# TuringLang/AdvancedVI.jl

Measured on AMD Instinct MI355X. Metric: ELBO-grad-estimates/sec, higher is better.
Workload: dtype f32

## Files before the change

advancedvi.jl_amd/csrc/api_batch.hip:

```cpp
#include "api_common.h"

mivi_status_t begin_capture(mivi_ctx *c, hipStream_t *saved) {
  if (!c->cap_stream) HIPCHK(c, hipStreamCreateWithFlags(&c->cap_stream, hipStreamNonBlocking));

  HIPCHK(c, hipStreamSynchronize(c->stream));
  *saved = c->stream;
  c->stream = c->cap_stream;
  hipError_t e = hipStreamBeginCapture(c->cap_stream, hipStreamCaptureModeThreadLocal);
  if (e != hipSuccess) { c->stream = *saved; c->err = std::string("hipStreamBeginCapture: ") + hipGetErrorString(e); return MIVI_ERR_HIP; }
  return MIVI_OK;
}
hipError_t end_capture(mivi_ctx *c, hipStream_t saved, hipGraph_t *graph) {
  hipError_t e = hipStreamEndCapture(c->cap_stream, graph);
  c->stream = saved;
  return e;
}

bool graph_capturable(const mivi_ctx *c) {
  return c->target == TGT_DIAG_GAUSS || c->target == TGT_DENSE_GAUSS || c->target == TGT_FUNNEL || c->target == TGT_LOGREG;
}
mivi_status_t reserve_target(mivi_ctx *c, int M) {
  if (c->target == TGT_LOGREG && !logreg_reserve(c, M)) return fail(c, MIVI_ERR_HIP, "logistic regression: scratch allocation failed");
  return MIVI_OK;
}

static mivi_status_t estimate_gradient_chain(mivi_ctx *c, const void *params, uint64_t idx0, int32_t count, void *value, void *grad) {
  if (!c || !params || !value || !grad || count <= 0) return MIVI_ERR_BAD_ARG;
  const uint64_t st = (uint64_t)c->idx_stride;
  if (!graph_capturable(c)) return fail(c, MIVI_ERR_UNSUPPORTED, "graph batching needs a device-resident built-in target");
  if (c->idx_src) return fail(c, MIVI_ERR_UNSUPPORTED, "an index source is set (mivi_set_index_source): graph-batched calls keep their own device counter");
  (void)hipSetDevice(c->cfg.device);
  mivi_status_t s = ensure_work(c, c->cfg.n_mc);
  if (s) return s;
  prepare_tables(c, c->cfg.n_mc);
  if ((s = reserve_target(c, c->cfg.n_mc))) return s;
  static const bool no_fused_loop_n = getenv("MIVI_NO_FUSED_LOOP") != nullptr;
  if (c->cfg.family == MIVI_MEANFIELD && c->target == TGT_DIAG_GAUSS && !c->bij_on && c->cfg.n_mc <= 4096 && !c->idx_src && !no_fused_loop_n) {
    const size_t hist_doubles = (size_t)count * 4 * (size_t)((c->cfg.d + 3) / 4);
    const size_t lane_bytes = (size_t)mf_loop_lanes(c, count) * 2 * (size_t)c->cfg.d * c->esize;
    if ((s = ensure(c, c->X, ((size_t)count + hist_doubles + 8) * sizeof(double) + lane_bytes, false))) return s;
    double *rec = (double *)c->X.p;
    launch_mf_sgd_loop(c, const_cast<void *>(params), nullptr, idx0, 0, count, -1, 0.0, (double)NAN, rec + count, rec, grad,
                       (void *)(rec + count + hist_doubles + 8), value);
    HIPCHK(c, hipGetLastError());
    return MIVI_OK;
  }
  if (c->cfg.family == MIVI_MEANFIELD && c->target == TGT_FUNNEL && !c->funnel_constrained && !c->bij_on && c->cfg.n_mc <= 256 && !c->idx_src &&
      !no_fused_loop_n) {
    const size_t d4 = (size_t)((c->cfg.d + 3) / 4);
    const size_t nd = (size_t)count * 6 * d4 + (size_t)count + 8;
    const size_t sc_bytes = ((size_t)count * ((size_t)c->cfg.d + 2) * c->esize + 63) & ~(size_t)63;
    const size_t lane_bytes = (size_t)mf_loop_lanes(c, count) * 2 * (size_t)c->cfg.d * c->esize;
    const size_t lane_al = (lane_bytes + 63) & ~(size_t)63;
    const size_t e0_bytes = (size_t)count * (size_t)c->cfg.n_mc * c->esize;
    if ((s = ensure(c, c->X, nd * sizeof(double) + sc_bytes + lane_al + e0_bytes + 64, false))) return s;
    double *hist = (double *)c->X.p, *elbo = hist + (size_t)count * 6 * d4;
    void *scratch = (void *)(elbo + count + 8);
    launch_mf_funnel_loop(c, params, idx0, count, hist, elbo, scratch, value, grad, (void *)((char *)scratch + sc_bytes),
                          (void *)((char *)scratch + sc_bytes + lane_al));
    HIPCHK(c, hipGetLastError());
    return MIVI_OK;
  }
  static const int graph_min = getenv("MIVI_GRAPH_MIN") ? atoi(getenv("MIVI_GRAPH_MIN")) : 6;
  if (count < graph_min && c->cfg.family == MIVI_FULLRANK) {
    Chain chn;
    chn.on = true;
    chn.estimates_only = true;
    for (int i = 0; i < count && s == MIVI_OK; ++i) {
      c->cur = i & 1;
      chn.has_next = (i + 1 < count);
      chn.next_rng = rng_of(c, idx0 + ((uint64_t)i + 1) * st);
      s = run_estimate(c, params, rng_of(c, idx0 + (uint64_t)i * st), c->cfg.n_mc, 1, final_out(c, value, grad), &chn);
    }
    if (s == MIVI_OK) flush_chain(c, params, &chn);
    c->cur = 0;
    c->pre_valid = false;
    if (s) return s;
    HIPCHK(c, hipGetLastError());
    return MIVI_OK;
  }
  GraphCache &g = c->graph;
  if (!(g.exec && g.kind == 1 && g.count == count && g.params == params && g.value == value && g.grad == grad)) {
    invalidate_graph(c);
    hipGraph_t graph = nullptr;
    hipStream_t saved;
    if ((s = begin_capture(c, &saved))) return s;
    Chain chn;
    chn.on = true;
    chn.estimates_only = true;
    for (int i = 0; i < count && s == MIVI_OK; ++i) {
      RngArgs r = rng_of(c, (uint64_t)i * st);
      r.idx_ptr = (const uint64_t *)c->d_idx.p;
      c->cur = i & 1;
      chn.has_next = (i + 1 < count);
      chn.next_rng = rng_of(c, ((uint64_t)i + 1) * st);
      chn.next_rng.idx_ptr = r.idx_ptr;
      s = run_estimate(c, params, r, c->cfg.n_mc, 1, final_out(c, value, grad), &chn);
    }
    if (s == MIVI_OK) flush_chain(c, params, &chn);
    if (s == MIVI_OK) hipLaunchKernelGGL(k_bump_u64, dim3(1), dim3(1), 0, c->stream, (uint64_t *)c->d_idx.p, (uint64_t)count * st);
    c->cur = 0;
    hipError_t e = end_capture(c, saved, &graph);
    if (s) { if (graph) (void)hipGraphDestroy(graph); return s; }
    HIPCHK(c, e);
    HIPCHK(c, hipGraphInstantiate(&g.exec, graph, nullptr, nullptr, 0));
    (void)hipGraphDestroy(graph);
    g.kind = 1; g.count = count; g.params = params; g.value = value; g.grad = grad;
  }
  if (!(c->d_idx_valid && c->d_idx_expect == idx0))
    hipLaunchKernelGGL(k_set_u64x2, dim3(1), dim3(1), 0, c->stream, (uint64_t *)c->d_idx.p, idx0, 0ull, 1);
  HIPCHK(c, hipGraphLaunch(g.exec, c->stream));
  c->d_idx_valid = true;
  c->d_idx_expect = idx0 + (uint64_t)count * st;
  return MIVI_OK;
}

static int chain_lanes() {
  static const int v = getenv("MIVI_CHAINS") ? atoi(getenv("MIVI_CHAINS")) : 0;
  return v;
}
mivi_status_t sync_kid(mivi_ctx *c, mivi_ctx *k, int lanes) {
  if (k->kid_gen == c->target_gen && k->idx_stride == lanes) return MIVI_OK;
  invalidate_graph(k);
  k->target = c->target;
  k->t_const = c->t_const;
  k->t_mean = c->t_mean; k->t_istd = c->t_istd; k->t_prec = c->t_prec;
  k->M_total = c->M_total;
  if (k->target == TGT_DENSE_GAUSS && !k->RT.p) k->cap_M = 0;
  k->idx_stride = lanes;
  k->kid_gen = c->target_gen;
  return MIVI_OK;
}

mivi_status_t ensure_kids(mivi_ctx *c, int lanes) {
  mivi_status_t s;
  while (c->n_kids < lanes - 1) {
    mivi_config_t cfg = c->cfg;
    cfg.stream = nullptr;
    cfg.own_stream = 1;
    mivi_ctx *k = nullptr;
    if ((s = mivi_create(&cfg, &k))) return fail(c, s, "interleaved chains: child context creation failed");
    k->is_child = true;
    const int j = c->n_kids;
    (void)hipFree(k->status.p);
    k->status.p = (char *)c->status.p + sizeof(int) * (j + 1);
    if ((s = ensure(c, c->kid_out[j], 16 + (size_t)mivi_params_len(c) * c->esize, false))) { (void)mivi_destroy(k); return s; }
    if (hipEventCreateWithFlags(&c->ev_join[j], hipEventDisableTiming) != hipSuccess ||
        (!c->ev_fork && hipEventCreateWithFlags(&c->ev_fork, hipEventDisableTiming) != hipSuccess)) {
      (void)hipGetLastError();
      (void)mivi_destroy(k);
      return fail(c, MIVI_ERR_HIP, "interleaved chains: event creation failed");
    }
    c->kids[c->n_kids++] = k;
  }
  return MIVI_OK;
}

static int fb_lanes_max() {
  static const int v = getenv("MIVI_FB_LANES") ? atoi(getenv("MIVI_FB_LANES")) : 80;
  return v < 1 ? 1 : (v > 256 ? 256 : v);
}
static bool fb_stl_on() {
  static const bool off = getenv("MIVI_FB_STL") && atoi(getenv("MIVI_FB_STL")) == 0;
  return !off;
}
static bool fb_route(const mivi_ctx *c, const void *params, const void *grad_last, const void *grads_all) {
  const bool stl = c->cfg.entropy == MIVI_ENT_STL || c->cfg.entropy == MIVI_ENT_STL_ZERO_GRAD;
  return !c->is_child && c->cfg.family == MIVI_FULLRANK && c->cfg.dtype == MIVI_F32 && !c->bij_on && !c->idx_src && !c->dbg &&
         (c->target == TGT_DIAG_GAUSS || c->target == TGT_DENSE_GAUSS) && (!stl || (fb_stl_on() && stl2_shape_ok(c, c->cfg.d))) &&
         fb_shape_ok(c, c->cfg.n_mc) && ((!stl && c->target == TGT_DIAG_GAUSS) || fb_whole_tiles(c, c->cfg.n_mc)) &&
         ((uintptr_t)params & 15) == 0 && ((uintptr_t)grad_last & 15) == 0 && ((uintptr_t)grads_all & 15) == 0;
}
static mivi_status_t fb_batch(mivi_ctx *c, const void *params, uint64_t idx0, int count, void *value_last, void *grad_last, void *values_all,
                              void *grads_all, int obj_ent = -1, bool dist = false) {
  mivi_status_t s;
  const int M = c->cfg.n_mc, d = c->cfg.d;
  if ((s = ensure_work(c, M))) return s;
  const bool overlap = dist && c->comm != nullptr;
  const int Lmax = (overlap && c->comm_world > 1) ? (fb_lanes_max() < 24 ? fb_lanes_max() : 24) : fb_lanes_max();
  const int steps = (count + Lmax - 1) / Lmax, L = (count + steps - 1) / steps, Llast = count - (steps - 1) * L;
  if (overlap && (s = dist_comm_stream(c))) return s;
  const size_t plen = (size_t)mivi_params_len(c);
  const int dG = (d + 127) / 128 * 128, MG = (M + 127) / 128 * 128;
  FbTables &t = c->fb;
  if (t.cap_L < L || t.cap_M != M) {
    invalidate_graph(c);
    const size_t pw = fb_plane_words(c, M) * 4;
    if ((s = ensure(c, t.CA, fb_cplane_words(c) * 4, false)) || (s = ensure(c, t.epsP, (size_t)L * pw, false)) ||
        (s = ensure(c, t.WV, (size_t)L * pw, false)) ||
        (s = ensure(c, t.ell, (size_t)L * (dG / 32) * (MG / 32) * sizeof(double), false)) ||
        (s = ensure(c, t.he, (size_t)L * (dG / 64) * (MG / 32) * sizeof(double), false)) ||
        (s = ensure(c, t.ld, 2 * (size_t)(dG / 32) * sizeof(double) + 64, false)) || (s = ensure(c, t.values, (size_t)L * 4 + 64, false)) ||
        (s = ensure(c, t.cscale, 2 * (size_t)dG * 4, false)) || (s = ensure(c, t.winv, (size_t)L * (MG / 128) * dG * 4, false)))
      return s;
    t.grads.bytes = 0;
    if ((s = ensure(c, t.grads, (size_t)L * plen * 4, true))) return s;
    t.cap_L = L;
    t.cap_M = M;
    t.cap_LR = 0;
  }
  const size_t part_len = dist ? fb_part_len(c) : 0;
  if (dist && t.cap_LP < L) {
    invalidate_graph(c);
    if ((s = ensure(c, t.parts, 2 * (size_t)L * part_len * 4, false))) return s;
    t.cap_LP = L;
  }
  const bool dense = c->target == TGT_DENSE_GAUSS;
  if (dense) {
    if (t.cap_LR < L) {
      invalidate_graph(c);
      if ((s = ensure(c, t.RP, (size_t)L * fb_plane_words(c, M) * 4, false)) || (s = ensure(c, t.PA, fb_cplane_words(c) * 4, false)) ||
          (s = ensure(c, t.pscale, 2 * (size_t)d * 4, false)) || (s = ensure(c, t.rinv, (size_t)L * (d / 128) * M * 4, false)))
        return s;
      t.cap_LR = L;
      t.PA_valid = false;
    }
    if (!t.PA_valid) {
      fb_launch_pplanes(c, c->stream);
      t.PA_valid = true;
    }
  }
  const bool values_only = obj_ent >= 0 || (!grads_all && !grad_last);
  const bool stl = !values_only && (c->cfg.entropy == MIVI_ENT_STL || c->cfg.entropy == MIVI_ENT_STL_ZERO_GRAD);
  if (stl) {
    const size_t es = 4;
    if (!t.Eye.p) {
      std::vector<float> eye((size_t)d * d, 0.f);
      for (int i = 0; i < d; ++i) eye[(size_t)i * d + i] = 1.f;
      if ((s = ensure(c, t.Eye, (size_t)d * d * es, false))) return s;
      HIPCHK(c, hipMemcpy(t.Eye.p, eye.data(), (size_t)d * d * es, hipMemcpyHostToDevice));
    }
    const bool grow = !t.Tinv.p || c->stl_X.bytes < ((size_t)d * d + (size_t)(d / 2) * (d / 2)) * es + 4096 || !c->stl_F.p;
    if (grow) {
      invalidate_graph(c);
      if ((s = ensure(c, t.Tinv, (size_t)d * d * es, false)) || (s = ensure(c, t.TA, fb_cplane_words(c) * 4, false)) || (s = ensure(c, t.tscale, 2 * (size_t)d * 4, false)) ||
          (s = ensure(c, c->stl_X, ((size_t)d * d + (size_t)(d / 2) * (d / 2)) * es + 4096, false)) ||
          (s = ensure(c, c->stl_F, mivi::stl_pack_units(d) * 4, false)))
        return s;
    }
    launch_stl2(c, params, d, false, t.Eye.p, t.Tinv.p, true);
    fb_launch_tplanes(c, c->stream);
  }
  const FbTab *tabF = fb_prepare(c, M, L), *tabL = Llast != L ? fb_prepare(c, M, Llast) : tabF;
  if (Llast != L) tabF = fb_prepare(c, M, L);
  if (!tabF || !tabL) return fail(c, MIVI_ERR_HIP, "batch engine: work table allocation failed");
  auto make_step = [&](int st) {
    FbStep fs{};
    fs.params = params;
    fs.M = M;
    fs.L = st == steps - 1 ? Llast : L;
    fs.tab = st == steps - 1 ? tabL : tabF;
    fs.rng = rng_of(c, obj_ent >= 0 ? idx0 : idx0 + (uint64_t)st * L);
    fs.obj = obj_ent >= 0 ? 1 : 0;
    fs.ent_kind = obj_ent;
    fs.values_only = values_only ? 1 : 0;
    if (obj_ent >= 0) fs.rng.m_offset += st * L * M;
    if (grads_all) { fs.grads = (char *)grads_all + (size_t)st * L * plen * 4; fs.grad_stride = (long long)plen; fs.write_upper = 1; }
    else { fs.grads = t.grads.p; fs.grad_stride = (long long)plen; fs.write_upper = 0; }
    if (values_all) { fs.values = (char *)values_all + (size_t)st * L * 4; fs.value_stride = 1; }
    else { fs.values = t.values.p; fs.value_stride = 1; }
    fs.lane_last = -1;
    fs.dense = dense ? 1 : 0;
    fs.stl = stl ? 1 : 0;
    if (st == steps - 1 && (value_last || grad_last)) { fs.lane_last = Llast - 1; fs.grad_last = grad_last; fs.value_last = value_last; }
    if (dist) { fs.parts = (char *)t.parts.p + (size_t)(overlap ? (st & 1) : 0) * (size_t)t.cap_LP * part_len * 4; fs.part_stride = (long long)part_len; }
    return fs;
  };
  for (int st = 0; st < steps; ++st) {
    const FbStep fs = make_step(st);
    const int b = st & 1;
    if (overlap && st >= 2) HIPCHK(c, hipStreamWaitEvent(c->stream, c->fb_ev_comm[b], 0));
    fb_launch_eps(c, fs, st == 0, c->stream);
    fb_launch_compute(c, fs, c->stream);
    if (dist) {
      hipStream_t xs = c->stream;
      if (overlap) {
        HIPCHK(c, hipEventRecord(c->fb_ev_part[b], c->stream));
        HIPCHK(c, hipStreamWaitEvent(c->fb_comm_stream, c->fb_ev_part[b], 0));
        xs = c->fb_comm_stream;
      }
      if ((s = dist_allreduce_f32(c, fs.parts, (size_t)fs.L * part_len, xs))) return s;
      fb_launch_finalize_parts(c, fs, xs);
      if (overlap) HIPCHK(c, hipEventRecord(c->fb_ev_comm[b], c->fb_comm_stream));
    }
  }
  if (overlap) {
    if (steps >= 2) HIPCHK(c, hipStreamWaitEvent(c->stream, c->fb_ev_comm[(steps - 2) & 1], 0));
    HIPCHK(c, hipStreamWaitEvent(c->stream, c->fb_ev_comm[(steps - 1) & 1], 0));
  }
  HIPCHK(c, hipGetLastError());
  return MIVI_OK;
}

mivi_status_t mivi::fb_objective(mivi_ctx *c, const void *params, uint64_t idx, int lanes, int entropy, void *values) {
  if (!fb_route(c, params, nullptr, nullptr) || c->M_total != c->cfg.n_mc) return MIVI_ERR_UNSUPPORTED;
  return fb_batch(c, params, idx, lanes, nullptr, nullptr, values, nullptr, entropy);
}

int32_t mivi_batch_lanes(const mivi_ctx_t *c, int32_t count) {
  if (!c || count <= 0) return 0;
  const int Lmax = fb_lanes_max(), steps = (count + Lmax - 1) / Lmax;
  return (count + steps - 1) / steps;
}

int32_t mivi_batch_info(const mivi_ctx_t *c, const void *params, int32_t what) {
  if (!c) return 0;
  if (what == 1) return 3;
  if (what == 2) return 4;
  if (what == 3) return c->exchange_lost ? 1 : 0;
  return (what == 0 && params && fb_route(c, params, nullptr, nullptr)) ? 1 : 0;
}

mivi_status_t mivi_profile_batch(mivi_ctx_t *c, const void *params, int32_t lanes, int32_t reps, double *us_out) {
  if (!c || !params || lanes <= 0 || reps <= 0 || !us_out) return MIVI_ERR_BAD_ARG;
  (void)hipSetDevice(c->cfg.device);
  if (!fb_route(c, params, nullptr, nullptr)) return fail(c, MIVI_ERR_UNSUPPORTED, "mivi_profile_batch: this configuration does not take the batch engine");
  if (lanes > fb_lanes_max()) lanes = fb_lanes_max();
  char *o = (char *)c->tmp_out.p;
  mivi_status_t s = fb_batch(c, params, 1, lanes, o, o + 16, nullptr, nullptr);
  if (s) return s;
  const FbTab *tab = fb_prepare(c, c->cfg.n_mc, lanes);
  if (!tab) return fail(c, MIVI_ERR_HIP, "batch engine: work table allocation failed");
  FbStep fs{};
  fs.params = params; fs.M = c->cfg.n_mc; fs.L = lanes; fs.tab = tab;
  fs.rng = rng_of(c, 1);
  fs.grads = c->fb.grads.p; fs.grad_stride = (long long)mivi_params_len(c); fs.values = c->fb.values.p; fs.value_stride = 1; fs.lane_last = -1;
  fs.dense = c->target == TGT_DENSE_GAUSS ? 1 : 0;
  fs.stl = (c->cfg.entropy == MIVI_ENT_STL || c->cfg.entropy == MIVI_ENT_STL_ZERO_GRAD) ? 1 : 0;
  us_out[3] = us_out[4] = 0.0;
  hipEvent_t e0, e1;
  HIPCHK(c, hipEventCreate(&e0));
  HIPCHK(c, hipEventCreate(&e1));
  for (int which = 0; which < 5; ++which) {
    if ((which == 3 && !fs.dense) || (which == 4 && !fs.stl)) continue;
    for (int r = -2; r < reps; ++r) {
      if (r == 0) HIPCHK(c, hipEventRecord(e0, c->stream));
      if (which == 0) fb_launch_eps(c, fs, true, c->stream);
      else fb_launch_compute(c, fs, c->stream, which == 1 ? 1 : (which == 2 ? 2 : (which == 3 ? 4 : 8)));
    }
    HIPCHK(c, hipEventRecord(e1, c->stream));
    HIPCHK(c, hipEventSynchronize(e1));
    float ms = 0.f;
    HIPCHK(c, hipEventElapsedTime(&ms, e0, e1));
    us_out[which] = (double)ms * 1e3 / reps;
  }
  (void)hipEventDestroy(e0);
  (void)hipEventDestroy(e1);
  HIPCHK(c, hipGetLastError());
  return MIVI_OK;
}

bool fb_dist_route(const mivi_ctx *c, const void *params, const void *grad) { return fb_route(c, params, grad, nullptr) && fb_whole_tiles(c, c->cfg.n_mc); }
mivi_status_t fb_batch_dist(mivi_ctx *c, const void *params, uint64_t idx0, int count, void *value, void *grad) {
  return fb_batch(c, params, idx0, count, value, grad, nullptr, nullptr, -1, true);
}

mivi_status_t mivi_estimate_gradient_each(mivi_ctx_t *c, const void *params, uint64_t idx0, int32_t count, void *values, void *grads) {
  if (!c || !params || !values || count <= 0) return MIVI_ERR_BAD_ARG;
  (void)hipSetDevice(c->cfg.device);
  if (c->target == TGT_NONE) return fail(c, MIVI_ERR_NO_TARGET, "no target set");
  if (fb_route(c, params, nullptr, grads)) return fb_batch(c, params, idx0, count, nullptr, nullptr, values, grads);
  const size_t plen = (size_t)mivi_params_len(c);
  mivi_status_t s = MIVI_OK;
  for (int i = 0; i < count && s == MIVI_OK; ++i)
    s = run_estimate(c, params, rng_of(c, idx0 + (uint64_t)i), c->cfg.n_mc, 1,
                     final_out(c, (char *)values + (size_t)i * c->esize, grads ? (void *)((char *)grads + (size_t)i * plen * c->esize) : c->tmp_out.p));
  return s;
}

mivi_status_t mivi_estimate_gradient_n(mivi_ctx_t *c, const void *params, uint64_t idx0, int32_t count, void *value, void *grad) {
  if (!c || !params || !value || !grad || count <= 0) return MIVI_ERR_BAD_ARG;
  (void)hipSetDevice(c->cfg.device);
  if (count >= 2 && fb_route(c, params, grad, nullptr)) return fb_batch(c, params, idx0, count, value, grad, nullptr, nullptr);
  int lanes = 1;
  if (!c->is_child && c->cfg.family == MIVI_FULLRANK && c->cfg.dtype == MIVI_F32 && !c->bij_on && !c->idx_src && !c->dbg &&
      (c->target == TGT_DIAG_GAUSS || c->target == TGT_DENSE_GAUSS) && lds_path_shape_ok(c, c->cfg.n_mc) &&
      (long long)c->cfg.d * c->cfg.n_mc <= 2048LL * 512)
    lanes = 4;
  static const int lane_env = getenv("MIVI_LANE_BATCH") ? atoi(getenv("MIVI_LANE_BATCH")) : -1;
  const bool stl_ent = c->cfg.entropy == MIVI_ENT_STL || c->cfg.entropy == MIVI_ENT_STL_ZERO_GRAD;
  int lane_e = 0;
  if (lanes > 1 && (!stl_ent || stl2_shape_ok(c, c->cfg.n_mc)) && lds_use_prod32(c, c->cfg.n_mc) && lds_bf16x3() && ((uintptr_t)params & 15) == 0 &&
      ((uintptr_t)grad & 15) == 0 && lane_env != 0) {
    lane_e = lane_env > 0 ? (lane_env > 4 ? 4 : lane_env) : 4;
    lanes = count < 12 ? 4 : 8;
  }
  if (chain_lanes() > 0) lanes = c->is_child ? 1 : (chain_lanes() > mivi_ctx::kMaxKids + 1 ? mivi_ctx::kMaxKids + 1 : chain_lanes());
  if (lane_e > 0 && (lanes % lane_e != 0 || count < lanes)) lane_e = 0;
  if (lane_e <= 0 && lanes > 4) lanes = 4;
  if (lane_e > 0 && lanes / lane_e > 4) lanes = 4 * lane_e;
  while (lanes > 1 && count < 4 * lanes && lane_e <= 0) --lanes;
  if (lanes <= 1) {
    if (!c->is_child && c->idx_stride != 1) { invalidate_graph(c); c->idx_stride = 1; }
    return estimate_gradient_chain(c, params, idx0, count, value, grad);
  }
  mivi_status_t s;
  if ((s = ensure_kids(c, lanes))) return s;
  if (c->idx_stride != lanes) { invalidate_graph(c); c->idx_stride = lanes; }
  for (int j = 0; j < lanes - 1; ++j)
    if ((s = sync_kid(c, c->kids[j], lanes))) return s;
  const int q_last = (count - 1) % lanes;
  if ((s = ensure_work(c, c->cfg.n_mc))) return s;
  prepare_tables(c, c->cfg.n_mc);
  for (int j = 0; j < lanes - 1; ++j) {
    mivi_ctx *k = c->kids[j];
    if ((s = ensure_work(k, k->cfg.n_mc))) { c->err = k->err; return s; }
    prepare_tables(k, k->cfg.n_mc);
    if (!lds_prepare(k, k->cfg.n_mc)) return fail(c, MIVI_ERR_HIP, "full-rank work lists: allocation failed");
  }
  if (!lds_prepare(c, c->cfg.n_mc)) return fail(c, MIVI_ERR_HIP, "full-rank work lists: allocation failed");
  GraphCache &g = c->graph;
  if (lane_e > 0) {
    const int lane_mode = lane_e;
    const int E = lane_mode, B = lanes / E;
    if (!(g.exec && g.kind == 3 && g.count == count && g.params == params && g.value == value && g.grad == grad && g.p0 == (double)(lanes * 16 + E))) {
      invalidate_graph(c);
      c->idx_stride = lanes;
      for (int j = 0; j < lanes - 1; ++j) {
        c->kids[j]->kid_gen = c->target_gen;
        HIPCHK(c, hipStreamSynchronize(c->kids[j]->stream));
      }
      hipGraph_t graph = nullptr;
      hipStream_t saved;
      if ((s = begin_capture(c, &saved))) return s;
      hipError_t he = hipEventRecord(c->ev_fork, c->stream);
      mivi_ctx *ctxs[1 + mivi_ctx::kMaxKids];
      ctxs[0] = c;
      for (int l = 1; l < lanes; ++l) ctxs[l] = c->kids[l - 1];
      const bool dense = c->target == TGT_DENSE_GAUSS;
      auto branch = [&](int b) -> mivi_status_t {
        mivi_status_t st = MIVI_OK;
        LaneSink *sink = lane_sinks_alloc(E);
        StlSink *ssink = stl_ent ? stl_sinks_alloc(E) : nullptr;
        EpsSink *esink = eps_sink_alloc();
        Chain chn[4];
        hipStream_t bs = ctxs[b * E]->stream, kept[4];
        mivi_ctx *lead = ctxs[b * E];
        for (int l = 0; l < E; ++l) {
          mivi_ctx *k = ctxs[b * E + l];
          kept[l] = k->stream;
          k->stream = bs;
          chn[l].on = true; chn[l].estimates_only = true;
          k->lane_sink = sink; k->lane_id = l;
          k->stl_sink = ssink;
          k->eps_sink = esink;
        }
        const int steps = (count + lanes - 1) / lanes;
        for (int i = 0; i < steps && st == MIVI_OK; ++i) {
          int L = 0;
          eps_sink_reset(esink);
          for (int l = 0; l < E && st == MIVI_OK; ++l) {
            const int gl = b * E + l;
            const int cnt = (count - gl + lanes - 1) / lanes;
            if (i >= cnt) break;
            mivi_ctx *k = ctxs[gl];
            lane_sink_reset(sink, l);
            if (ssink) stl_sink_reset(ssink, l);
            RngArgs r = rng_of(k, (uint64_t)gl + (uint64_t)i * lanes);
            r.idx_ptr = (const uint64_t *)c->d_idx.p;
            k->cur = i & 1;
            chn[l].has_next = (i + 1 < cnt);
            chn[l].next_rng = rng_of(k, (uint64_t)gl + ((uint64_t)i + 1) * lanes);
            chn[l].next_rng.idx_ptr = r.idx_ptr;
            char *ko = gl ? (char *)c->kid_out[gl - 1].p : (char *)c->tmp_out.p;
            st = run_estimate(k, params, r, k->cfg.n_mc, 1, final_out(k, gl == q_last ? value : (void *)ko, gl == q_last ? grad : (void *)(ko + 16)), &chn[l]);
            if (st) { c->err = k->err; break; }
            if (lane_sink_counts(sink, l) != (dense ? 2 : 1) * 16 + 1 || (ssink && stl_sink_count(ssink, l) != 1))
              st = fail(c, MIVI_ERR_HIP, "lane-batched estimates: an estimate did not take the expected kernel route");
            ++L;
          }
          if (st == MIVI_OK && L > 0) launch_lanes_eps(lead, esink, L);
          if (st == MIVI_OK && L > 0 && !(launch_lanes_prod(lead, sink, L, 0) && (!dense || launch_lanes_prod(lead, sink, L, 1)) &&
                                          (!ssink || launch_lanes_stl(lead, ssink, L, i == 0)) && launch_lanes_vjp(lead, sink, L)))
            st = fail(c, MIVI_ERR_HIP, "lane-batched estimates: the lanes' launches do not match");
        }
        ValueSink *vsink = value_sink_alloc();
        for (int l = 0; l < E; ++l) {
          mivi_ctx *k = ctxs[b * E + l];
          k->lane_sink = nullptr;
          k->stl_sink = nullptr;
          k->eps_sink = nullptr;
          k->value_sink = vsink;
          if (st == MIVI_OK) flush_chain(k, params, &chn[l]);
          k->value_sink = nullptr;
          k->cur = 0;
          k->pre_valid = false;
        }
        if (st == MIVI_OK) launch_lanes_value(lead, params, vsink);
        value_sink_free(vsink);
        for (int l = 0; l < E; ++l) ctxs[b * E + l]->stream = kept[l];
        lane_sinks_free(sink);
        if (ssink) stl_sinks_free(ssink);
        eps_sink_free(esink);
        return st;
      };
      for (int b = 1; b < B && s == MIVI_OK && he == hipSuccess; ++b) {
        mivi_ctx *k = ctxs[b * E];
        he = hipStreamWaitEvent(k->stream, c->ev_fork, 0);
        if (he != hipSuccess) break;
        s = branch(b);
        if (s == MIVI_OK) he = hipEventRecord(c->ev_join[b * E - 1], k->stream);
      }
      if (s == MIVI_OK && he == hipSuccess) s = branch(0);
      for (int b = 1; b < B && s == MIVI_OK && he == hipSuccess; ++b) he = hipStreamWaitEvent(c->stream, c->ev_join[b * E - 1], 0);
      if (s == MIVI_OK && he == hipSuccess) hipLaunchKernelGGL(k_bump_u64, dim3(1), dim3(1), 0, c->stream, (uint64_t *)c->d_idx.p, (uint64_t)count);
      hipError_t e = end_capture(c, saved, &graph);
      if (s) { if (graph) (void)hipGraphDestroy(graph); return s; }
      HIPCHK(c, he);
      HIPCHK(c, e);
      HIPCHK(c, hipGraphInstantiate(&g.exec, graph, nullptr, nullptr, 0));
      (void)hipGraphDestroy(graph);
      g.kind = 3; g.count = count; g.params = params; g.value = value; g.grad = grad; g.p0 = (double)(lanes * 16 + E);
    }
    if (!(c->d_idx_valid && c->d_idx_expect == idx0))
      hipLaunchKernelGGL(k_set_u64x2, dim3(1), dim3(1), 0, c->stream, (uint64_t *)c->d_idx.p, idx0, 0ull, 1);
    HIPCHK(c, hipGraphLaunch(g.exec, c->stream));
    c->d_idx_valid = true;
    c->d_idx_expect = idx0 + (uint64_t)count;
    return MIVI_OK;
  }
  if (!(g.exec && g.kind == 2 && g.count == count && g.params == params && g.value == value && g.grad == grad && g.p0 == (double)lanes)) {
    invalidate_graph(c);
    c->idx_stride = lanes;
    for (int j = 0; j < lanes - 1; ++j) {
      c->kids[j]->kid_gen = c->target_gen;
      HIPCHK(c, hipStreamSynchronize(c->kids[j]->stream));
    }
    hipGraph_t graph = nullptr;
    hipStream_t saved;
    if ((s = begin_capture(c, &saved))) return s;
    hipError_t he = hipEventRecord(c->ev_fork, c->stream);
    auto chain_body = [&](mivi_ctx *k, int q, int cnt, void *v, void *gr) -> mivi_status_t {
      Chain chn;
      chn.on = true;
      chn.estimates_only = true;
      mivi_status_t st = MIVI_OK;
      for (int i = 0; i < cnt && st == MIVI_OK; ++i) {
        RngArgs r = rng_of(k, (uint64_t)q + (uint64_t)i * lanes);
        r.idx_ptr = (const uint64_t *)c->d_idx.p;
        k->cur = i & 1;
        chn.has_next = (i + 1 < cnt);
        chn.next_rng = rng_of(k, (uint64_t)q + ((uint64_t)i + 1) * lanes);
        chn.next_rng.idx_ptr = r.idx_ptr;
        st = run_estimate(k, params, r, k->cfg.n_mc, 1, final_out(k, v, gr), &chn);
      }
      if (st == MIVI_OK) flush_chain(k, params, &chn);
      k->cur = 0;
      k->pre_valid = false;
      return st;
    };
    for (int q = 1; q < lanes && s == MIVI_OK && he == hipSuccess; ++q) {
      mivi_ctx *k = c->kids[q - 1];
      char *ko = (char *)c->kid_out[q - 1].p;
      he = hipStreamWaitEvent(k->stream, c->ev_fork, 0);
      if (he != hipSuccess) break;
      s = chain_body(k, q, (count - q + lanes - 1) / lanes, q == q_last ? value : (void *)ko, q == q_last ? grad : (void *)(ko + 16));
      if (s) c->err = k->err;
      if (s == MIVI_OK) he = hipEventRecord(c->ev_join[q - 1], k->stream);
    }
    if (s == MIVI_OK && he == hipSuccess) {
      char *ko = (char *)c->tmp_out.p;
      s = chain_body(c, 0, (count + lanes - 1) / lanes, q_last == 0 ? value : (void *)ko, q_last == 0 ? grad : (void *)(ko + 16));
    }
    for (int q = 1; q < lanes && s == MIVI_OK && he == hipSuccess; ++q) he = hipStreamWaitEvent(c->stream, c->ev_join[q - 1], 0);
    if (s == MIVI_OK && he == hipSuccess) hipLaunchKernelGGL(k_bump_u64, dim3(1), dim3(1), 0, c->stream, (uint64_t *)c->d_idx.p, (uint64_t)count);
    hipError_t e = end_capture(c, saved, &graph);
    if (s) { if (graph) (void)hipGraphDestroy(graph); return s; }
    HIPCHK(c, he);
    HIPCHK(c, e);
    HIPCHK(c, hipGraphInstantiate(&g.exec, graph, nullptr, nullptr, 0));
    (void)hipGraphDestroy(graph);
    g.kind = 2; g.count = count; g.params = params; g.value = value; g.grad = grad; g.p0 = (double)lanes;
  }
  if (!(c->d_idx_valid && c->d_idx_expect == idx0))
    hipLaunchKernelGGL(k_set_u64x2, dim3(1), dim3(1), 0, c->stream, (uint64_t *)c->d_idx.p, idx0, 0ull, 1);
  HIPCHK(c, hipGraphLaunch(g.exec, c->stream));
  c->d_idx_valid = true;
  c->d_idx_expect = idx0 + (uint64_t)count;
  return MIVI_OK;
}
```

advancedvi.jl_amd/csrc/api_core.hip:

```cpp
#include "api_common.h"

__global__ void k_acc_value_f32(double *acc, const float *v, double w, int first) { acc[0] = (first ? 0.0 : acc[0]) + w * (double)v[0]; }
__global__ void k_acc_value_f64(double *acc, const double *v, double w, int first) { acc[0] = (first ? 0.0 : acc[0]) + w * v[0]; }
__global__ void k_store_value_f32(float *out, const double *acc) { out[0] = (float)acc[0]; }
__global__ __launch_bounds__(256) void k_mean_values_f32(double *acc, const float *v, int n, double w) {
  __shared__ double part[256];
  double s = 0.0;
  for (int i = threadIdx.x; i < n; i += 256) s += (double)v[i];
  part[threadIdx.x] = s;
  __syncthreads();
  if (threadIdx.x == 0) {
    double t = 0.0;
    for (int i = 0; i < 256; ++i) t += part[i];
    acc[0] = w * t;
  }
}
__global__ void k_store_value_f64(double *out, const double *acc) { out[0] = acc[0]; }
__global__ void k_set_u64x2(uint64_t *dst, uint64_t a, uint64_t b, int n) { dst[0] = a; if (n > 1) dst[1] = b; }
__global__ void k_bump_u64(uint64_t *dst, uint64_t by) { dst[0] += by; }
__global__ void k_empty(int *sink) {
  extern __shared__ int lds_dyn[];
  if (sink && threadIdx.x == 0 && blockIdx.x == 0x7fffffff) sink[0] = lds_dyn[0];
}


mivi_status_t fail(mivi_ctx *c, mivi_status_t s, const char *msg) {
  if (c) c->err = msg;
  return s;
}

namespace mivi {
bool grid_resident(const mivi_ctx *c, const void *kernel, int block, size_t dyn_lds, long long grid) {
  int nb = 0;
  if (hipOccupancyMaxActiveBlocksPerMultiprocessor(&nb, kernel, block, dyn_lds) != hipSuccess) { (void)hipGetLastError(); return false; }
  return c->n_cu > 0 && (long long)nb * c->n_cu >= grid;
}
}

mivi_status_t ensure(mivi_ctx *c, DevBuf &b, size_t bytes, bool zero) {
  if (b.bytes >= bytes && b.p) return MIVI_OK;
  if (b.p) HIPCHK(c, hipFree(b.p));
  b.p = nullptr;
  b.bytes = 0;
  if (bytes == 0) bytes = 16;
  HIPCHK(c, hipMalloc(&b.p, bytes));
  b.bytes = bytes;
  if (zero) HIPCHK(c, hipMemsetAsync(b.p, 0, bytes, c->stream));
  return MIVI_OK;
}


namespace mivi {
void invalidate_graph(mivi_ctx *c) {
  c->pre_valid = false;
  ++c->target_gen;
  if (c->graph.exec) { (void)hipGraphExecDestroy(c->graph.exec); c->graph = GraphCache{}; }
}
}

mivi_status_t ensure_work(mivi_ctx *c, int M) {
  const int d = c->cfg.d;
  const size_t es = c->esize;
  mivi_status_t s;
  if (M > c->cap_M) {
    invalidate_graph(c);
    const int capM = round_up(M, 64);
    c->dP = round_up(d, 64);
    c->MP = capM;
    const int d4 = (d + 3) / 4;
    size_t n_part = 8 * (size_t)(((d + 31) / 32 + 7) / 8) * (size_t)((capM + 31) / 32) + 64;
    size_t n_he = (size_t)((d + 15) / 16) * (size_t)(capM / 64 + 1);
    const size_t n_he_mf = (size_t)((d4 + 255) / 256) * (size_t)capM;
    if (n_he_mf > n_he) n_he = n_he_mf;
    const size_t ncc = (size_t)(capM / 256 + 2);
    for (int b = 0; b < 2; ++b) {
      if (c->cfg.family == MIVI_FULLRANK) {
        c->eps[b].bytes = 0; c->epsT[b].bytes = 0;
        if ((s = ensure(c, c->eps[b], (size_t)c->dP * c->MP * es, true))) return s;
        if ((s = ensure(c, c->epsT[b], (size_t)c->dP * c->MP * es, true))) return s;
      }
      if ((s = ensure(c, c->ell_part[b], n_part * sizeof(double), false))) return s;
      if ((s = ensure(c, c->he_part[b], (n_he + 64) * sizeof(double), false))) return s;
      if ((s = ensure(c, c->sc_part[b], 6 * ncc * d4 * sizeof(double) + 64, false))) return s;
      if ((s = ensure(c, c->ld_part[b], 2 * (size_t)((d + 31) / 32) * sizeof(double) + 64, false))) return s;
    }
    if (c->target == TGT_DENSE_GAUSS || (c->target == TGT_LOGREG && c->cfg.dtype == MIVI_F32)) {
      c->RT.bytes = 0;
      if ((s = ensure(c, c->RT, (size_t)c->dP * c->MP * es, true))) return s;
    }
    if (c->cfg.family == MIVI_FULLRANK && (c->cfg.entropy == MIVI_ENT_STL || c->cfg.entropy == MIVI_ENT_STL_ZERO_GRAD)) {
      if ((s = ensure(c, c->stl_CT, (size_t)c->dP * c->dP * es, true))) return s;
      if ((s = ensure(c, c->stl_Dinv, (size_t)((d + 63) / 64) * 4096 * es, false))) return s;
      if ((s = ensure(c, c->stl_X, ((size_t)d * capM + (size_t)(d / 2) * (d / 2)) * es + 4096, false))) return s;
      if (d % 128 == 0 && (s = ensure(c, c->stl_F, mivi::stl_pack_units(d) * 4, false))) return s;
    }
    if ((s = ensure(c, c->Z, (size_t)d * capM * es, false))) return s;
    if ((s = ensure(c, c->W, (size_t)d * capM * es, false))) return s;
    if ((s = ensure(c, c->ell, (size_t)capM * es, false))) return s;
    if (c->bij_on && (s = ensure(c, c->bij_ld, (size_t)capM * es, false))) return s;
    if ((s = ensure(c, c->row_part, ncc * d4 * 8 * sizeof(double), false))) return s;
    c->cap_M = capM;
  }
  return MIVI_OK;
}


int32_t mivi_version(void) { return MIVI_VERSION_MAJOR * 1000 + MIVI_VERSION_MINOR; }

const char *mivi_last_error(const mivi_ctx_t *ctx) { return ctx ? ctx->err.c_str() : "null context"; }

int64_t mivi_params_len(const mivi_ctx_t *c) {
  const int64_t d = c->cfg.d;
  return c->cfg.family == MIVI_MEANFIELD ? 2 * d : d + d * d;
}
int64_t mivi_partials_len(const mivi_ctx_t *c) {
  const int64_t d = c->cfg.d;
  return (c->cfg.family == MIVI_MEANFIELD ? 2 * d : d + d * (d + 1) / 2) + 2;
}

mivi_status_t mivi_create(const mivi_config_t *cfg, mivi_ctx_t **out) {
  if (!cfg || !out) return MIVI_ERR_BAD_ARG;
  if (cfg->d <= 0 || cfg->n_mc <= 0) return MIVI_ERR_BAD_ARG;
  if (cfg->dtype != MIVI_F32 && cfg->dtype != MIVI_F64) return MIVI_ERR_BAD_ARG;
  if (cfg->family != MIVI_MEANFIELD && cfg->family != MIVI_FULLRANK) return MIVI_ERR_BAD_ARG;
  if (cfg->entropy < 0 || cfg->entropy > MIVI_ENT_STL_ZERO_GRAD) return MIVI_ERR_BAD_ARG;
  if (cfg->m_offset < 0) return MIVI_ERR_BAD_ARG;
  int ndev = 0;
  if (hipGetDeviceCount(&ndev) != hipSuccess || ndev <= 0 || cfg->device < 0 || cfg->device >= ndev) {
    fprintf(stderr, "libmivi: no usable HIP device %d (found %d): this library has no CPU fallback\n", cfg->device, ndev);
    return MIVI_ERR_HIP;
  }
  mivi_ctx *c = new mivi_ctx();
  c->cfg = *cfg;
  c->esize = cfg->dtype == MIVI_F32 ? 4 : 8;
  {
    int v = 0;
    if (hipDeviceGetAttribute(&v, hipDeviceAttributeMultiprocessorCount, cfg->device) == hipSuccess && v > 0) c->n_cu = v;
    if (hipDeviceGetAttribute(&v, hipDeviceAttributeMaxSharedMemoryPerBlock, cfg->device) == hipSuccess && v > 0) c->lds_max = (size_t)v;
    (void)hipGetLastError();
  }
  c->M_total = cfg->m_total > 0 ? cfg->m_total : cfg->n_mc;
  if (hipSetDevice(cfg->device) != hipSuccess) { delete c; return MIVI_ERR_HIP; }
  if (!cfg->own_stream) {
    c->stream = (hipStream_t)cfg->stream;
  } else {
    if (hipStreamCreateWithFlags(&c->stream, hipStreamNonBlocking) != hipSuccess) { delete c; return MIVI_ERR_HIP; }
    c->own_stream = true;
  }
  mivi_status_t s;
  if ((s = ensure(c, c->status, 64, true)) ||
      (s = ensure(c, c->d_idx, 64, true)) || (s = ensure(c, c->acc, 64, true)) ||
      (s = ensure(c, c->dog_part, (2 * 512 + 8) * sizeof(double), true)) ||
      (s = ensure(c, c->tmp_params, (size_t)mivi_params_len(c) * c->esize, false)) ||
      (s = ensure(c, c->tmp_out, ((size_t)mivi_params_len(c) + 16) * c->esize, false))) {
    delete c;
    return s;
  }
  *out = c;
  return MIVI_OK;
}

mivi_status_t mivi_destroy(mivi_ctx_t *c) {
  if (!c) return MIVI_ERR_BAD_ARG;
  (void)hipSetDevice(c->cfg.device);
  (void)hipStreamSynchronize(c->stream);
  for (int j = 0; j < c->n_kids; ++j) {
    (void)mivi_destroy(c->kids[j]);
    if (c->ev_join[j]) (void)hipEventDestroy(c->ev_join[j]);
    if (c->kid_out[j].p) (void)hipFree(c->kid_out[j].p);
  }
  if (c->ev_fork) (void)hipEventDestroy(c->ev_fork);
  if (c->is_child) c->t_mean = c->t_istd = c->t_prec = c->status = mivi::DevBuf{};
  (void)mivi_comm_destroy(c);
  if (c->graph.exec) (void)hipGraphExecDestroy(c->graph.exec);
  DevBuf *bufs[] = {&c->t_mean, &c->t_istd, &c->t_prec, &c->lr_X_own, &c->lr_y_own, &c->lr_scratch, &c->lr_part, &c->lr_Xrm,
                    &c->eps[0], &c->eps[1], &c->epsT[0], &c->epsT[1], &c->Z, &c->W, &c->RT, &c->ell, &c->X,
                    &c->ell_part[0], &c->ell_part[1], &c->he_part[0], &c->he_part[1], &c->row_part,
                    &c->sc_part[0], &c->sc_part[1], &c->ld_part[0], &c->ld_part[1], &c->tabA, &c->tabB, &c->tabD, &c->stl_CT, &c->stl_Dinv, &c->stl_X, &c->stl_F, &c->lr_xmax, &c->lr_XA, &c->lr_XB, &c->lr_ZP, &c->lr_Xsub, &c->lr_ysub, &c->lr_Xrm_sub, &c->lr_idx, &c->dog_part, &c->stein_A, &c->stein_g, &c->h2_acc, &c->bij_mask, &c->bij_ld, &c->dist_P, &c->dist_P2, &c->dist_ring[0], &c->dist_ring[1], &c->dist_ring[2], &c->dist_ring[3], &c->dist_ring[4], &c->dist_ring[5], &c->p2p_scratch, &c->dist_S, &c->dist_F, &c->p2p_tab, &c->p2p_ctr, &c->lds_tabV, &c->lds_tabV64, &c->lds_tabS, &c->lds_tabSt, &c->status, &c->d_idx, &c->acc, &c->tmp_params, &c->tmp_out, &c->obj_vals};
  for (DevBuf *b : bufs)
    if (b->p) (void)hipFree(b->p);
  {
    DevBuf *fbb[] = {&c->fb.CA, &c->fb.epsP, &c->fb.WV, &c->fb.ell, &c->fb.he, &c->fb.ld, &c->fb.grads, &c->fb.values, &c->fb.PA, &c->fb.RP, &c->fb.Tinv, &c->fb.TA, &c->fb.Eye, &c->snap, &c->fb.cscale, &c->fb.pscale, &c->fb.tscale, &c->fb.winv, &c->fb.rinv, &c->p2p_direct, &c->rows_eps, &c->gen_scratch};
    for (DevBuf *b : fbb)
      if (b->p) (void)hipFree(b->p);
    for (auto &tb : c->fb.tab) {
      if (tb.prod.p) (void)hipFree(tb.prod.p);
      if (tb.vjp.p) (void)hipFree(tb.vjp.p);
      if (tb.prod2.p) (void)hipFree(tb.prod2.p);
      if (tb.prod3.p) (void)hipFree(tb.prod3.p);
    }
  }
  if (c->own_stream) (void)hipStreamDestroy(c->stream);
  if (c->cap_stream) (void)hipStreamDestroy(c->cap_stream);
  if (c->comm_stream) (void)hipStreamDestroy(c->comm_stream);
  if (c->comm_stream2) (void)hipStreamDestroy(c->comm_stream2);
  if (c->fb_comm_stream) (void)hipStreamDestroy(c->fb_comm_stream);
  for (int k = 0; k < 2; ++k) {
    if (c->fb_ev_part[k]) (void)hipEventDestroy(c->fb_ev_part[k]);
    if (c->fb_ev_comm[k]) (void)hipEventDestroy(c->fb_ev_comm[k]);
  }
  for (int k = 0; k < 2; ++k) {
    if (c->ev_part[k]) (void)hipEventDestroy(c->ev_part[k]);
    if (c->ev_comm[k]) (void)hipEventDestroy(c->ev_comm[k]);
  }
  delete c;
  return MIVI_OK;
}

mivi_status_t mivi_set_stream(mivi_ctx_t *c, void *s) {
  if (!c) return MIVI_ERR_BAD_ARG;
  if (c->own_stream) { (void)hipStreamSynchronize(c->stream); (void)hipStreamDestroy(c->stream); c->own_stream = false; }
  c->stream = (hipStream_t)s;
  c->pre_valid = false;
  if (c->graph.exec) { (void)hipGraphExecDestroy(c->graph.exec); c->graph = GraphCache{}; }
  return MIVI_OK;
}


mivi_status_t mivi_synchronize(mivi_ctx_t *c) {
  if (!c) return MIVI_ERR_BAD_ARG;
  return read_status(c);
}

double host_get(const void *p, int dtype, size_t i) {
  return dtype == MIVI_F32 ? (double)((const float *)p)[i] : ((const double *)p)[i];
}
static mivi_status_t upload_vec(mivi_ctx *c, DevBuf &b, const std::vector<double> &v) {
  mivi_status_t s = ensure(c, b, v.size() * c->esize, false);
  if (s) return s;
  if (c->cfg.dtype == MIVI_F32) {
    std::vector<float> f(v.begin(), v.end());
    HIPCHK(c, hipMemcpy(b.p, f.data(), f.size() * 4, hipMemcpyHostToDevice));
  } else {
    HIPCHK(c, hipMemcpy(b.p, v.data(), v.size() * 8, hipMemcpyHostToDevice));
  }
  return MIVI_OK;
}

mivi_status_t mivi_set_target_diag_gauss(mivi_ctx_t *c, const void *mean, const void *stdv) {
  if (!c || !mean || !stdv) return MIVI_ERR_BAD_ARG;
  (void)hipSetDevice(c->cfg.device);
  const int d = c->cfg.d;
  std::vector<double> m(d), is(d);
  double cst = -0.5 * d * kLog2Pi;
  for (int i = 0; i < d; ++i) {
    const double s = host_get(stdv, c->cfg.dtype, i);
    if (!(s > 0.0)) return fail(c, MIVI_ERR_BAD_ARG, "diag_gauss: std must be positive");
    m[i] = host_get(mean, c->cfg.dtype, i);
    is[i] = 1.0 / s;
    cst -= log(s);
  }
  mivi_status_t s;
  if ((s = upload_vec(c, c->t_mean, m)) || (s = upload_vec(c, c->t_istd, is))) return s;
  c->t_const = cst;
  c->target = TGT_DIAG_GAUSS;
  invalidate_graph(c);
  return MIVI_OK;
}

mivi_status_t mivi_set_target_dense_gauss(mivi_ctx_t *c, const void *mean, const void *Lh) {
  if (!c || !mean || !Lh) return MIVI_ERR_BAD_ARG;
  (void)hipSetDevice(c->cfg.device);
  const int d = c->cfg.d;
  const int dP = round_up(d, 64);
  std::vector<double> L((size_t)d * d, 0.0), Li((size_t)d * d, 0.0), m(d);
  double logdet = 0.0;
  for (int j = 0; j < d; ++j)
    for (int i = j; i < d; ++i) L[(size_t)j * d + i] = host_get(Lh, c->cfg.dtype, (size_t)j * d + i);
  for (int i = 0; i < d; ++i) {
    m[i] = host_get(mean, c->cfg.dtype, i);
    const double lii = L[(size_t)i * d + i];
    if (!(lii > 0.0)) return fail(c, MIVI_ERR_BAD_ARG, "dense_gauss: Cholesky diagonal must be positive");
    logdet += 2.0 * log(lii);
  }
  for (int j = 0; j < d; ++j) {
    Li[(size_t)j * d + j] = 1.0 / L[(size_t)j * d + j];
    for (int i = j + 1; i < d; ++i) {
      double s = 0.0;
      for (int k = j; k < i; ++k) s += L[(size_t)k * d + i] * Li[(size_t)j * d + k];
      Li[(size_t)j * d + i] = -s / L[(size_t)i * d + i];
    }
  }
  std::vector<double> P((size_t)dP * dP, 0.0);
  for (int i = 0; i < d; ++i)
    for (int j = 0; j <= i; ++j) {
      double s = 0.0;
      for (int k = i; k < d; ++k) s += Li[(size_t)i * d + k] * Li[(size_t)j * d + k];
      P[(size_t)j * dP + i] = s;
      P[(size_t)i * dP + j] = s;
    }
  mivi_status_t s;
  if ((s = upload_vec(c, c->t_mean, m)) || (s = upload_vec(c, c->t_prec, P))) return s;
  c->t_const = -0.5 * logdet - 0.5 * d * kLog2Pi;
  c->target = TGT_DENSE_GAUSS;
  c->fb.PA_valid = false;
  c->cap_M = 0;
  invalidate_graph(c);
  return MIVI_OK;
}

mivi_status_t mivi_set_target_logreg(mivi_ctx_t *c, const void *X, const uint8_t *y, int64_t n, int32_t variant,
                                     double likeadj, int32_t on_device) {
  if (!c || !X || !y || n <= 0 || (variant != 0 && variant != 1) || c->cfg.d < 2) return MIVI_ERR_BAD_ARG;
  (void)hipSetDevice(c->cfg.device);
  const int p = c->cfg.d - 1;
  if (on_device) {
    c->lr_X = X;
    c->lr_y = y;
  } else {
    mivi_status_t s;
    if ((s = ensure(c, c->lr_X_own, (size_t)n * p * c->esize, false)) || (s = ensure(c, c->lr_y_own, (size_t)n, false)))
      return s;
    HIPCHK(c, hipMemcpy(c->lr_X_own.p, X, (size_t)n * p * c->esize, hipMemcpyHostToDevice));
    HIPCHK(c, hipMemcpy(c->lr_y_own.p, y, (size_t)n, hipMemcpyHostToDevice));
    c->lr_X = c->lr_X_own.p;
    c->lr_y = (const uint8_t *)c->lr_y_own.p;
  }
  c->lr_n = n;
  c->lr_variant = variant;
  c->lr_likeadj = likeadj;
  c->lr_X_full = c->lr_X;
  c->lr_y_full = c->lr_y;
  c->lr_n_full = n;
  c->lr_likeadj_full = likeadj;
  c->t_const = 0.0;
  c->target = TGT_LOGREG;
  c->cap_M = 0;
  if (c->cfg.dtype == MIVI_F32 && !logreg_prepare_f32(c)) return fail(c, MIVI_ERR_HIP, "logistic regression: row-major copy allocation failed");
  c->lr_Xrm_act = c->cfg.dtype == MIVI_F32 ? c->lr_Xrm.p : nullptr;
  invalidate_graph(c);
  return MIVI_OK;
}

mivi_status_t mivi_logreg_select_rows(mivi_ctx_t *c, const int64_t *idx, int64_t b, double likeadj) {
  if (!c || b < 0 || (b > 0 && !idx)) return MIVI_ERR_BAD_ARG;
  if (c->target != TGT_LOGREG || !c->lr_X_full) return fail(c, MIVI_ERR_NO_TARGET, "no logistic-regression target set");
  (void)hipSetDevice(c->cfg.device);
  invalidate_graph(c);
  if (b == 0) {
    c->lr_X = c->lr_X_full;
    c->lr_y = c->lr_y_full;
    c->lr_n = c->lr_n_full;
    c->lr_likeadj = c->lr_likeadj_full;
    c->lr_Xrm_act = c->cfg.dtype == MIVI_F32 ? c->lr_Xrm.p : nullptr;
    return MIVI_OK;
  }
  if (!(likeadj > 0.0)) return fail(c, MIVI_ERR_BAD_ARG, "likelihood adjustment must be positive");
  for (int64_t j = 0; j < b; ++j)
    if (idx[j] < 0 || idx[j] >= c->lr_n_full) return fail(c, MIVI_ERR_BAD_ARG, "batch row index out of range");
  const int p = c->cfg.d - 1;
  mivi_status_t s;
  if ((s = ensure(c, c->lr_idx, (size_t)b * sizeof(int64_t), false)) ||
      (s = ensure(c, c->lr_Xsub, (size_t)b * p * c->esize, false)) || (s = ensure(c, c->lr_ysub, (size_t)b, false)))
    return s;
  if (c->cfg.dtype == MIVI_F32 && (s = ensure(c, c->lr_Xrm_sub, (size_t)((b + 15) / 16 * 16) * ((p + 31) / 32 * 32) * sizeof(float), false))) return s;
  HIPCHK(c, hipStreamSynchronize(c->stream));
  HIPCHK(c, hipMemcpy(c->lr_idx.p, idx, (size_t)b * sizeof(int64_t), hipMemcpyHostToDevice));
  launch_logreg_gather(c, b);
  HIPCHK(c, hipGetLastError());
  c->lr_X = c->lr_Xsub.p;
  c->lr_y = (const uint8_t *)c->lr_ysub.p;
  c->lr_n = b;
  c->lr_likeadj = likeadj;
  c->lr_Xrm_act = c->cfg.dtype == MIVI_F32 ? c->lr_Xrm_sub.p : nullptr;
  return MIVI_OK;
}

mivi_status_t mivi_set_target_funnel_constrained(mivi_ctx_t *c, double sigma_v) {
  mivi_status_t s = mivi_set_target_funnel(c, sigma_v);
  if (s == MIVI_OK) c->funnel_constrained = 1;
  return s;
}

mivi_status_t mivi_set_bijector_stacked(mivi_ctx_t *c, int32_t n_blocks, const int32_t *ranges, const int32_t *kinds) {
  if (!c || n_blocks < 0 || (n_blocks > 0 && (!ranges || !kinds))) return MIVI_ERR_BAD_ARG;
  (void)hipSetDevice(c->cfg.device);
  const int d = c->cfg.d;
  std::vector<uint8_t> mask(d, 0), seen(d, 0);
  bool any = false;
  for (int b = 0; b < n_blocks; ++b) {
    const int lo = ranges[2 * b], hi = ranges[2 * b + 1];
    if (lo < 0 || hi > d || lo > hi) return fail(c, MIVI_ERR_BAD_ARG, "stacked bijector: block range outside [0, d)");
    if (kinds[b] != 0 && kinds[b] != 1) return fail(c, MIVI_ERR_BAD_ARG, "stacked bijector: kind must be 0 (identity) or 1 (exp)");
    for (int i = lo; i < hi; ++i) {
      if (seen[i]) return fail(c, MIVI_ERR_BAD_ARG, "stacked bijector: blocks overlap");
      seen[i] = 1;
      mask[i] = (uint8_t)kinds[b];
      any = any || kinds[b] == 1;
    }
  }
  invalidate_graph(c);
  HIPCHK(c, hipStreamSynchronize(c->stream));
  if (!any) {
    c->bij_on = false;
    return MIVI_OK;
  }
  mivi_status_t s = ensure(c, c->bij_mask, (size_t)d, false);
  if (s) return s;
  HIPCHK(c, hipMemcpy(c->bij_mask.p, mask.data(), (size_t)d, hipMemcpyHostToDevice));
  c->bij_on = true;
  c->cap_M = 0;
  return MIVI_OK;
}

mivi_status_t mivi_set_target_funnel(mivi_ctx_t *c, double sigma_v) {
  if (!c || !(sigma_v > 0.0) || c->cfg.d < 2) return MIVI_ERR_BAD_ARG;
  c->funnel_constrained = 0;
  c->funnel_sigma_v = sigma_v;
  c->t_const = -log(sigma_v) - 0.5 * kLog2Pi - 0.5 * (c->cfg.d - 1) * kLog2Pi;
  c->target = TGT_FUNNEL;
  invalidate_graph(c);
  return MIVI_OK;
}

mivi_status_t mivi_set_target_callback(mivi_ctx_t *c, mivi_logdensity_and_gradient_fn fg, mivi_logdensity_fn fv,
                                       void *user) {
  if (!c || !fg) return MIVI_ERR_BAD_ARG;
  c->cb_grad = fg;
  c->cb_value = fv;
  c->cb_user = user;
  c->t_const = 0.0;
  c->target = TGT_CALLBACK;
  invalidate_graph(c);
  return MIVI_OK;
}

int32_t mivi_fullrank_route(const mivi_ctx_t *c, int32_t n_samples) {
  if (!c || c->cfg.family != MIVI_FULLRANK) return 0;
  if (n_samples <= 0) n_samples = c->cfg.n_mc;
  if (!lds_path_shape_ok(c, n_samples) || (c->target != TGT_DIAG_GAUSS && c->target != TGT_DENSE_GAUSS)) return 0;
  return (lds_use_prod32(c, n_samples) ? 1 : 3) | (lds_bf16x3() ? 16 : 0);
}

int32_t mivi_logreg_kernels(const mivi_ctx_t *c, int32_t n_samples) {
  if (!c) return 0;
  return logreg_kernel_bits(c, n_samples > 0 ? n_samples : c->cfg.n_mc);
}

mivi_status_t mivi_set_logreg_route(mivi_ctx_t *c, int32_t route) {
  if (!c || route < 0 || route > 2) return MIVI_ERR_BAD_ARG;
  c->lr_route = route;
  invalidate_graph(c);
  return MIVI_OK;
}

mivi_status_t mivi_set_index_source(mivi_ctx_t *c, const uint64_t *idx_dev) {
  if (!c) return MIVI_ERR_BAD_ARG;
  c->idx_src = idx_dev;
  invalidate_graph(c);
  return MIVI_OK;
}

mivi_status_t mivi_debug_timeline(mivi_ctx_t *c, void *buf) {
  if (!c) return MIVI_ERR_BAD_ARG;
#ifdef MIVI_DEV
  c->dbg = (long long *)buf;
  invalidate_graph(c);
  return MIVI_OK;
#else
  if (!buf) return MIVI_OK;
  return fail(c, MIVI_ERR_UNSUPPORTED, "timeline stamps are compiled out of the release library (build with `make DEV=1`)");
#endif
}

void mivi_philox4x32_10(const uint32_t ctr[4], const uint32_t key[2], uint32_t out[4]) {
  u32x4 c{ctr[0], ctr[1], ctr[2], ctr[3]};
  const u32x4 r = philox4x32_10(c, key[0], key[1]);
  out[0] = r.x; out[1] = r.y; out[2] = r.z; out[3] = r.w;
}

void mivi_eps_bits_host(uint64_t seed, uint64_t idx, int32_t d, int64_t m, int32_t i0, int32_t count, uint32_t *out) {
  const uint64_t d4 = (uint64_t)((d + 3) / 4);
  for (int32_t t = 0; t < count; ++t) {
    const int32_t i = i0 + t;
    const u32x4 b = eps_block_bits(seed, idx, (uint64_t)m * d4 + (uint64_t)(i / 4));
    const uint32_t w[4] = {b.x, b.y, b.z, b.w};
    out[t] = w[i & 3];
  }
}

void mivi_eps_host(uint64_t seed, uint64_t idx, int32_t d, int64_t m, int32_t i0, int32_t count, int32_t dtype,
                   double *out) {
  const uint64_t d4 = (uint64_t)((d + 3) / 4);
  for (int32_t t = 0; t < count; ++t) {
    const int32_t i = i0 + t;
    const uint64_t q = (uint64_t)m * d4 + (uint64_t)(i / 4);
    if (dtype == MIVI_F32) {
      float e[4];
      eps_block<float>(seed, idx, q, e);
      out[t] = (double)e[i & 3];
    } else {
      double e[4];
      eps_block<double>(seed, idx, q, e);
      out[t] = e[i & 3];
    }
  }
}
```

advancedvi.jl_amd/csrc/fr_elem.h:

```cpp
#pragma once
#include "device_common.h"

namespace mivi {

__device__ __forceinline__ float diag_target_elem(float z, float tm, float tis, float &ell) {
#pragma clang fp contract(off)
  const float u = (z - tm) * tis;
  ell = __builtin_fmaf(-0.5f * u, u, ell);
  return -u * tis;
}

__device__ __forceinline__ float dense_target_elem(float pr, float r, float &ell) {
#pragma clang fp contract(off)
  const float g = -pr;
  ell = __builtin_fmaf(0.5f * r, g, ell);
  return g;
}

__device__ __forceinline__ float vjp_elem(float v, int gi, int gj, bool pow2M, float invMf, double invM, double direct, float cjj) {
#pragma clang fp contract(off)
  if (gj > gi) return 0.f;
  if (pow2M && gj != gi) return -v * invMf;
  double x = -(double)v * invM;
  if (gj == gi) {
    const double q = direct / (double)cjj;
    x = x - q;
  }
  return (float)x;
}

__device__ __forceinline__ float dmu_elem(double sm, double invM) {
#pragma clang fp contract(off)
  return (float)(-sm * invM);
}

__device__ __forceinline__ void logdet_block32(float cii, float &lg, float &bad) {
  lg = logf(cii);
  bad = (cii > 0.f) ? 0.f : 1.f;
#pragma unroll
  for (int o = 16; o > 0; o >>= 1) {
    lg += __shfl_xor(lg, o, 64);
    bad += __shfl_xor(bad, o, 64);
  }
}

}
```

advancedvi.jl_amd/csrc/kernels_fullrank_batch.hip:

```cpp
#include <algorithm>
#include <cstdlib>
#include <type_traits>
#include <cstdio>
#include <vector>

#include "device_common.h"
#include "fr_elem.h"
#include "fr_planes.h"

#ifndef FB_VK
#define FB_VK 0
#endif
#ifndef FB_WJ
#define FB_WJ 1
#endif

namespace mivi {

struct FbArgs {
  int d, M, L;
  int dT, MT;
  const float *params;
  const float *t_mean, *t_istd;
  unsigned *CA;
  float *cscale;
  unsigned *epsP;
  unsigned *WV;
  float *winv;
  const float *t_prec;
  int dP;
  unsigned *PA;
  float *pscale;
  unsigned *RP;
  float *rinv;
  const float *Tinv;
  unsigned *TA;
  float *tscale;
  long long plane_stride;
  double *ell_part;
  long long ell_stride;
  double *he_part;
  long long he_stride;
  double *ld_part;
  const int4 *work;
  int n_work;
  float *grads;
  long long grad_stride;
  float *values;
  long long value_stride;
  float *grad_last, *value_last;
  int lane_last;
  int write_upper;
  int ent_kind, M_total;
  int *status;
  double ell_const;
  RngArgs rng;
  int n_riders;
  int obj;
  float *parts;
  long long part_stride;
  int knock;
  long long *dbg;
};
#ifdef MIVI_DEV
#define FB_STAMP(a, slot) do { if ((a).dbg && threadIdx.x == 0) (a).dbg[(size_t)blockIdx.x * 8 + (slot)] = (long long)wall_clock64(); } while (0)
#define FB_NOTE(a, slot, v) do { if ((a).dbg && threadIdx.x == 0) (a).dbg[(size_t)blockIdx.x * 8 + (slot)] = (long long)(v); } while (0)
#define FB_KNOCKED(a, b) ((a).knock & (b))
#else
#define FB_KNOCKED(a, b) false
#define FB_STAMP(a, slot) do { } while (0)
#define FB_NOTE(a, slot, v) do { } while (0)
#endif

template <class Ld4, class Ld>
__device__ __forceinline__ void fb_rowblock_planes(int d, int rb, int kg_lo, int kg_hi, int sub, int nsub, Ld4 ld4, Ld ld, unsigned *planes, float *scale, float *red) {
  const int tid = threadIdx.x, r4 = tid & 7, part = tid >> 3, ng = d >> 4;
  f32x4 m = {0.f, 0.f, 0.f, 0.f};
  {
    int k = 16 * kg_lo + part;
    for (; k + 448 <= 16 * kg_hi + 15; k += 512) {
      f32x4 v[8];
#pragma unroll
      for (int u = 0; u < 8; ++u) v[u] = ld4(k + 64 * u, 32 * rb + 4 * r4);
#pragma unroll
      for (int u = 0; u < 8; ++u)
#pragma unroll
        for (int c = 0; c < 4; ++c) m[c] = fmaxf(m[c], fabsf(v[u][c]));
    }
    for (; k <= 16 * kg_hi + 15; k += 64) {
      const f32x4 v = ld4(k, 32 * rb + 4 * r4);
#pragma unroll
      for (int c = 0; c < 4; ++c) m[c] = fmaxf(m[c], fabsf(v[c]));
    }
  }
#pragma unroll
  for (int c = 0; c < 4; ++c) {
    m[c] = fmaxf(m[c], __shfl_xor(m[c], 8, 64));
    m[c] = fmaxf(m[c], __shfl_xor(m[c], 16, 64));
    m[c] = fmaxf(m[c], __shfl_xor(m[c], 32, 64));
  }
  if ((tid & 63) < 8) *(f32x4 *)(red + (tid >> 6) * 32 + 4 * r4) = m;
  lds_barrier();
  if (tid < 32) {
    float mm = red[tid];
#pragma unroll
    for (int p = 1; p < 8; ++p) mm = fmaxf(mm, red[p * 32 + tid]);
    float s, inv;
    fb_scale_of(mm, s, inv);
    red[512 + tid] = s;
    if (sub == 0) {
      scale[32 * rb + tid] = s;
      scale[d + 32 * rb + tid] = inv;
    }
  }
  lds_barrier();
  const int w = tid >> 6, lane = tid & 63, l31 = lane & 31, h = lane >> 5;
  const float s = red[512 + l31];
  for (int kg = kg_lo + w + 8 * sub; kg <= kg_hi; kg += 8 * nsub) {
    float x[8];
#pragma unroll
    for (int e = 0; e < 8; ++e) x[e] = ld(16 * kg + 8 * (e >> 2) + 4 * h + (e & 3), 32 * rb + l31) * s;
    fb_store_frag(planes + ((size_t)rb * ng + kg) * kFrag + 4 * lane, x);
  }
}
__device__ __forceinline__ void fb_cplanes_block(const FbArgs &a, int rb, int sub, int nsub, float *red) {
  const int d = a.d, ng = d >> 4, dT = a.dT;
  const float *C = a.params + dT;
  const int hi = 2 * rb + 3 < ng - 1 ? 2 * rb + 3 : ng - 1;
  if (dT == d) {
    fb_rowblock_planes(d, rb, 0, hi, sub, nsub,
                       [C, d](int k, int row) { f32x4 v = *(const f32x4 *)(C + (size_t)k * d + row);
#pragma unroll
                                                for (int c = 0; c < 4; ++c) v[c] = k > row + c ? 0.f : v[c];
                                                return v; },
                       [C, d](int k, int row) { const float v = C[(size_t)k * d + row]; return k > row ? 0.f : v; }, a.CA, a.cscale, red);
    return;
  }
  fb_rowblock_planes(d, rb, 0, hi, sub, nsub,
                     [C, dT](int k, int row) { const bool in = row < dT && k < dT;
                                               f32x4 v = *(const f32x4 *)(C + (size_t)(in ? k : 0) * dT + (in ? row : 0));
#pragma unroll
                                               for (int c = 0; c < 4; ++c) v[c] = (!in || k > row + c) ? 0.f : v[c];
                                               return v; },
                     [C, dT](int k, int row) { if (row >= dT || k > row) return 0.f; return C[(size_t)k * dT + row]; }, a.CA, a.cscale, red);
}
__global__ __launch_bounds__(512) void k_fb_pplanes(FbArgs a) {
  __shared__ float red[16 * 32 + 32];
  const float *P = a.t_prec;
  const int dP = a.dP;
  fb_rowblock_planes(a.d, (int)blockIdx.x, 0, (a.d >> 4) - 1, (int)blockIdx.y, (int)gridDim.y,
                     [P, dP](int k, int row) { return *(const f32x4 *)(P + (size_t)k * dP + row); },
                     [P, dP](int k, int row) { return P[(size_t)k * dP + row]; }, a.PA, a.pscale, red);
}
__global__ __launch_bounds__(512) void k_fb_tplanes(FbArgs a) {
  __shared__ float red[16 * 32 + 32];
  const float *T = a.Tinv;
  const int d = a.d, rb = (int)blockIdx.x;
  fb_rowblock_planes(d, rb, 2 * (rb & ~3), (d >> 4) - 1, (int)blockIdx.y, (int)gridDim.y,
                     [T, d](int k, int row) { f32x4 v = *(const f32x4 *)(T + (size_t)k * d + row);
#pragma unroll
                                              for (int c = 0; c < 4; ++c) v[c] = k >= row + c ? v[c] : 0.f;
                                              return v; },
                     [T, d](int k, int row) { const float v = T[(size_t)k * d + row]; return k >= row ? v : 0.f; }, a.TA, a.tscale, red);
}

__global__ __launch_bounds__(512) void k_fb_eps(FbArgs a) {
  __shared__ double red[8];
  __shared__ float E[32 * 65];
  const int tid = threadIdx.x, eb = blockIdx.x, d = a.d;
  if ((int)blockIdx.y < a.n_riders) {
    const int r = (int)blockIdx.y * (int)gridDim.x + eb;
    if (r < 4 * (d >> 5)) fb_cplanes_block(a, (d >> 5) - 1 - (r >> 2), r & 3, 4, E);
    return;
  }
  const int l = (int)blockIdx.y - a.n_riders;
  const uint64_t idx = rng_index(a.rng) + (a.obj ? 0ull : (uint64_t)l);
  const int moff = a.rng.m_offset + (a.obj ? l * a.MT : 0);
  unsigned *epsP = a.epsP + (size_t)l * a.plane_stride;
  const int nrb6 = d >> 6;
  const int R64 = eb % nrb6, c32 = eb / nrb6;
  const int q = tid & 15, c = tid >> 4;
  const int ri = R64 * 64 + 4 * q, rm = c32 * 32 + c;
  float e[4];
  eps_block<float>(a.rng.seed, idx, (uint64_t)(moff + rm) * (uint64_t)(a.dT >> 2) + (uint64_t)(ri >> 2), e);
  if (!(ri < a.dT && rm < a.MT)) { e[0] = 0.f; e[1] = 0.f; e[2] = 0.f; e[3] = 0.f; }
#pragma unroll
  for (int r = 0; r < 4; ++r) E[c * 65 + 4 * q + r] = e[r] * kEpsScale;
  const float he = 0.5f * (e[0] * e[0] + e[1] * e[1] + e[2] * e[2] + e[3] * e[3]);
  const double sh = block_sum_nodrain_f32<512>(he, red);
  if (tid == 0) a.he_part[(size_t)l * a.he_stride + eb] = sh;
  if (tid >= 256) return;
  const int lane = tid & 63, l31 = lane & 31, h = lane >> 5, f = tid >> 6;
  float x[8];
#pragma unroll
  for (int s = 0; s < 8; ++s) x[s] = E[l31 * 65 + 16 * f + 8 * (s >> 2) + 4 * h + (s & 3)];
  fb_store_frag(epsP + ((size_t)c32 * (d >> 4) + 4 * R64 + f) * kFrag + 4 * lane, x);
}

constexpr int kImgW = 32 * 36;
template <int WJ>
__device__ __forceinline__ void fb_sched_interleave() {
  constexpr int NM = 6 * WJ, ND = 4 + 2 * WJ, NV = 2 * WJ;
  static_for<0, NM>([&](auto K) {
    constexpr int k = decltype(K)::value;
    constexpr int nrd = (k + 1) * ND / NM - k * ND / NM;
    __builtin_amdgcn_sched_group_barrier(0x008, 1, 0);
    if constexpr (nrd > 0) __builtin_amdgcn_sched_group_barrier(0x100, nrd, 0);
    if constexpr (k < NV) __builtin_amdgcn_sched_group_barrier(0x020, 1, 0);
  });
}
using FbI0 = std::integral_constant<int, 0>;
using FbI1 = std::integral_constant<int, 1>;
using FbI2 = std::integral_constant<int, 2>;
using FbI3 = std::integral_constant<int, 3>;
using FbT = std::true_type;
using FbN = std::false_type;

template <int MASK>
__device__ __forceinline__ float fb_lane_max(float v) {
#pragma unroll
  for (int o = 1; o < 64; o <<= 1)
    if (MASK & o) v = fmaxf(v, __shfl_xor(v, o, 64));
  return v;
}

enum { FB_DIAG = 0, FB_DENSE_R = 1, FB_DENSE_G = 2, FB_STL_U = 3 };
template <int WJ, int MODE, int NRP>
__global__ __launch_bounds__(512 / WJ, (MODE == 2 && NRP == 4 && WJ == 1) ? 4 : 2 / WJ) void k_fb_prod(FbArgs a) {
  constexpr bool kDG = MODE == FB_DENSE_G, kSU = MODE == FB_STL_U, kDR = MODE == FB_DENSE_R;
  constexpr int LDC = 36, NF = WJ, kPW = 2 * WJ;
  constexpr int NW = 8 / WJ, NWN = 4 / WJ;
  constexpr int kBody = (NRP * kStageW > 16 * kImgW) ? NRP * kStageW : 16 * kImgW;
  constexpr bool kTabInBody = kDG && NRP * kStageW + 2048 <= kBody;
  constexpr int kTab = kDG ? (kTabInBody ? 128 : 2048 + 128) : 0;
  __shared__ __attribute__((aligned(16))) unsigned lds[kBody + 4 * 128 + NW * 64 + kTab];
  float *vec = reinterpret_cast<float *>(lds + kBody);
  float *red = vec + 4 * 128;
  float *rsv = red + NW * 64;
  float *tab = kTabInBody ? reinterpret_cast<float *>(lds + NRP * kStageW) : rsv + 128;
  const int tid = threadIdx.x, lane = tid & 63, l31 = lane & 31, h = lane >> 5;
  const int w = __builtin_amdgcn_readfirstlane(tid >> 6);
  const int wm = w / NWN, wn = w % NWN;
  const __attribute__((address_space(4))) int *wp = (const __attribute__((address_space(4))) int *)a.work + 4 * blockIdx.x;
  const int ln = wp[0], rc = wp[1], flags = wp[2];
  const int rb = rc & 0xffff, cb = rc >> 16;
  const int d = a.d, ng = d >> 4;
  const int row0 = rb * 128, col0 = cb * 128;
  const int R0 = row0 >> 5;
  const int g0 = kSU ? 2 * R0 : 0;
  const int G = kDG ? ng : (kSU ? ng - g0 : 2 * (R0 + 4));
  const unsigned *sp[NF];
  int gmax[NF];
#pragma unroll
  for (int f = 0; f < NF; ++f) {
    const int fs = NF * w + f, fr = fs & 3;
    if (fs < 4) {
      sp[f] = (kDG ? a.PA : (kSU ? a.TA : a.CA)) + ((size_t)(R0 + fr) * ng + g0) * kFrag + 4 * lane;
      gmax[f] = (!kDG && !kSU && 2 * (R0 + fr) + 3 < G - 1) ? 2 * (R0 + fr) + 3 : G - 1;
    } else {
      sp[f] = (kDG ? a.RP : a.epsP) + (size_t)ln * a.plane_stride + ((size_t)((col0 >> 5) + fr) * ng + g0) * kFrag + 4 * lane;
      gmax[f] = G - 1;
    }
  }
  int gd = 0;
  constexpr int kMaxNB = 16;
  float tv[4] = {0.f, 0.f, 0.f, 0.f}, tri[kDG ? kMaxNB : 1], trs = 0.f;
  auto load_tables = [&]() {
    if (tid < 128) {
      if constexpr (!kDG && !kSU) {
        const bool in = row0 + tid < a.dT;
        tv[0] = in ? a.params[row0 + tid] : 0.f;
        tv[1] = in ? a.t_mean[row0 + tid] : 0.f;
        if (MODE == FB_DIAG) tv[2] = in ? a.t_istd[row0 + tid] : 0.f;
      }
      const float *sc = kDG ? a.pscale : (kSU ? a.tscale : a.cscale);
      tv[3] = sc[d + row0 + tid];
      if constexpr (kDG) {
        const float *ri = a.rinv + (size_t)ln * (size_t)(d >> 7) * a.M + col0 + tid;
        const int NB = d >> 7;
#pragma unroll
        for (int b = 0; b < kMaxNB; ++b) tri[b] = ri[(size_t)(b < NB ? b : NB - 1) * a.M];
        trs = ri[(size_t)rb * a.M];
      }
    }
    asm volatile("" ::: "memory");
  };
  auto stage_tables = [&]() {
    if (tid < 128) {
      if constexpr (!kDG && !kSU) {
        vec[tid] = tv[0];
        vec[128 + tid] = tv[1];
        if (MODE == FB_DIAG) vec[256 + tid] = tv[2];
      }
      vec[384 + tid] = tv[3] * ((kDG) ? 1.f : kEpsInv);
      if constexpr (kDG) {
        const int NB = d >> 7;
        float u = tri[0], grow = 1.f;
#pragma unroll
        for (int b = 1; b < kMaxNB; ++b) {
          if (b < NB) {
            float ratio = u / tri[b];
            if (!(ratio <= 1099511627776.f)) ratio = 1099511627776.f;
            if (ratio > 1.f && grow * ratio > 1.2089258e24f) ratio = fmaxf(1.2089258e24f / grow, 1.f);
            if (ratio > 1.f) grow *= ratio;
            tab[(b - 1) * 128 + tid] = ratio;
            u = u / ratio;
          }
        }
        tab[(NB - 1) * 128 + tid] = u;
        rsv[tid] = trs;
      }
    }
  };
  auto issue = [&](int slot) {
#pragma unroll
    for (int f = 0; f < NF; ++f) {
      unsigned *dst = lds + slot * kStageW + (NF * w + f) * 512;
      FB_GLDS16(sp[f], dst, 0);
      FB_GLDS16(sp[f], dst, 1024);
      sp[f] += gd < gmax[f] ? kFrag : 0;
    }
    ++gd;
  };
  f32x16 acc[2][WJ];
#pragma unroll
  for (int i = 0; i < 2; ++i)
#pragma unroll
    for (int j = 0; j < WJ; ++j)
#pragma unroll
      for (int r = 0; r < 16; ++r) acc[i][j][r] = 0.f;
  const int r32[2] = {R0 + 2 * wm, R0 + 2 * wm + 1};
  const int Gw = (kDG || kSU) ? G : 2 * r32[1] + 2;
  auto after_group = [&](auto S, int g) {
    if constexpr (kDG && (decltype(S)::value & 3) == 3) {
      if (((g + 1) & 7) == 0) {
#pragma unroll
        for (int j = 0; j < WJ; ++j) {
          const float f = tab[((g >> 3) << 7) + 32 * (WJ * wn + j) + l31];
#pragma unroll
          for (int i = 0; i < 2; ++i) {
#pragma unroll
            for (int r = 0; r < 16; ++r) acc[i][j][r] *= f;
          }
        }
        asm volatile("" ::: "memory");
      }
    }
  };
  auto compute = [&](auto S, int g, const FbFrags<WJ> &F) {
    if (!FB_KNOCKED(a, 2)) fb_group<WJ>(F, acc);
    fb_sched_interleave<WJ>();
    after_group(S, g);
  };
  const unsigned lds0 = (unsigned)(uintptr_t)lds + 16u * lane;
  const unsigned ab_lo = lds0 + (2 * wm) * 2 * 1024, bb_lo = lds0 + (8 + WJ * wn * 2) * 1024;
  const unsigned ab_hi = ab_lo + 4 * kStageW * 4, bb_hi = bb_lo + 4 * kStageW * 4;
  (void)ab_hi; (void)bb_hi;
  auto step = [&](auto S, auto VM, auto ISS, int g, const FbFrags<WJ> &Fc, FbFrags<WJ> &Fn) {
    constexpr int sl = decltype(S)::value;
    fb_wait_vm<kPW * decltype(VM)::value>();
    if (!FB_KNOCKED(a, 8)) fb_barrier();
#ifdef MIVI_SB
    __builtin_amdgcn_sched_barrier(0);
#endif
    auto group_and_read = [&]() {
#ifndef MIVI_DEV
      if constexpr (WJ == 1) {
        constexpr int nx = (sl + 1) % NRP, off = (nx & 3) * kStageW * 4;
        fb_group_read_asm<off>(acc[0][0], acc[1][0], Fc, Fn, nx < 4 ? ab_lo : ab_hi, nx < 4 ? bb_lo : bb_hi);
        if constexpr (kDG && (sl & 3) == 3) {
          if (((g + 1) & 7) == 0) asm volatile("s_nop 15\n\ts_nop 7" : "+v"(acc[0][0]), "+v"(acc[1][0])::"memory");
        }
        after_group(S, g);
      } else
#endif
      {
        if (!FB_KNOCKED(a, 4)) fb_read_frags<WJ>(lds, (sl + 1) % NRP, wm, wn, lane, Fn);
        compute(S, g, Fc);
      }
    };
    if constexpr (decltype(ISS)::value) {
      if (!FB_KNOCKED(a, 1)) issue(sl);
      group_and_read();
    } else if (g < Gw) {
      group_and_read();
    }
  };
  FB_STAMP(a, 0);
  FB_NOTE(a, 4, G);
  load_tables();
  static_for<0, NRP>([&](auto S) { issue(decltype(S)::value); });
  fb_wait_vm<kPW * NRP>();
  stage_tables();
  fb_wait_vm<kPW * (NRP - 1)>();
  fb_barrier();
  FB_STAMP(a, 1);
  {
    FbFrags<WJ> F0, F1;
    fb_read_frags<WJ>(lds, 0, wm, wn, lane, F0);
    int g = 0;
    for (; g + NRP < G; g += NRP) {
      static_for<0, NRP>([&](auto S) {
        constexpr int sv = decltype(S)::value;
        if constexpr (sv % 2 == 0) step(S, std::integral_constant<int, NRP - 2>{}, FbT{}, g + sv, F0, F1);
        else step(S, std::integral_constant<int, NRP - 2>{}, FbT{}, g + sv, F1, F0);
      });
    }
    static_for<0, NRP - 1>([&](auto S) {
      constexpr int sv = decltype(S)::value;
      if constexpr (sv % 2 == 0) step(S, std::integral_constant<int, NRP - 2 - sv>{}, FbN{}, g + sv, F0, F1);
      else step(S, std::integral_constant<int, NRP - 2 - sv>{}, FbN{}, g + sv, F1, F0);
    });
    __builtin_amdgcn_s_waitcnt(0xc07f);
    if (g + NRP - 1 < Gw) compute(std::integral_constant<int, NRP - 1>{}, g + NRP - 1, F1);
  }
  f32x16 (&tot)[2][WJ] = acc;
  fb_barrier();
  FB_STAMP(a, 2);
  float *img = reinterpret_cast<float *>(lds) + w * (2 * WJ * kImgW);
  unsigned *WVl = a.WV + (size_t)ln * a.plane_stride;
  unsigned *RPl = a.RP + (size_t)ln * a.plane_stride;
  double *ellp = a.ell_part + (size_t)ln * a.ell_stride;
  const int ncb = a.M >> 5, nmg = a.M >> 4;
  const int ei4 = 4 * (lane & 7);
  float amax[2][4];
  float cmax[WJ][4];
#pragma unroll
  for (int i = 0; i < 2; ++i)
#pragma unroll
    for (int c = 0; c < 4; ++c) amax[i][c] = 0.f;
#pragma unroll
  for (int j = 0; j < WJ; ++j)
#pragma unroll
    for (int p = 0; p < 4; ++p) cmax[j][p] = 0.f;
#pragma unroll
  for (int i = 0; i < 2; ++i) {
    const int lr = 64 * wm + 32 * i;
    f32x4 mu = {0.f, 0.f, 0.f, 0.f}, tm = mu, tis = mu;
    const f32x4 zf = *(const f32x4 *)(vec + 384 + lr + ei4);
    if constexpr (!kDG && !kSU) {
      mu = *(const f32x4 *)(vec + lr + ei4);
      tm = *(const f32x4 *)(vec + 128 + lr + ei4);
      if constexpr (MODE == FB_DIAG) tis = *(const f32x4 *)(vec + 256 + lr + ei4);
    }
#pragma unroll
    for (int j = 0; j < WJ; ++j) {
      float *I = img + (i * WJ + j) * kImgW;
      const int cb32 = (col0 >> 5) + WJ * wn + j;
      const bool pad = 32 * r32[i] >= a.dT || 32 * cb32 >= a.MT;
#pragma unroll
      for (int q = 0; q < 4; ++q) {
        const f32x4 v = {tot[i][j][4 * q], tot[i][j][4 * q + 1], tot[i][j][4 * q + 2], tot[i][j][4 * q + 3]};
        *(f32x4 *)(I + l31 * LDC + 8 * q + 4 * h) = v;
      }
      if constexpr (kSU) {
        const float uf = vec[384 + lr + l31];
        const float wo = a.winv[(size_t)ln * (size_t)(a.M >> 7) * d + (size_t)cb * d + row0 + lr + l31];
#pragma unroll
        for (int g2 = 0; g2 < 2; ++g2) {
          const unsigned *src = WVl + ((size_t)r32[i] * nmg + 2 * cb32 + g2) * kFrag + 4 * lane;
          const u32x4v wh = *(const u32x4v *)src, wl = *(const u32x4v *)(src + 256);
#pragma unroll
          for (int e = 0; e < 8; ++e) {
            float *p = I + (16 * g2 + 8 * (e >> 2) + 4 * h + (e & 3)) * LDC + l31;
            const float x = __builtin_fmaf(*p, uf, fb_unsplit2(wh, wl, e) * wo);
            *p = x;
            amax[i][0] = fmaxf(amax[i][0], fabsf(x));
          }
        }
        continue;
      }
      double s = 0.0;
#pragma unroll
      for (int p = 0; p < 4; ++p) {
        const int en = 8 * p + (lane >> 3);
        const f32x4 v = *(const f32x4 *)(I + en * LDC + ei4) * zf;
        float ell = 0.f;
        f32x4 wv;
        if constexpr (MODE == FB_DIAG) {
          const f32x4 z = mu + v;
#pragma unroll
          for (int c = 0; c < 4; ++c) wv[c] = diag_target_elem(z[c], tm[c], tis[c], ell);
        } else if constexpr (kDR) {
          const f32x4 z = mu + v;
          wv = z - tm;
        } else {
          const unsigned *fr = RPl + ((size_t)cb32 * ng + 2 * r32[i] + (ei4 >> 4)) * kFrag + 4 * (en + 32 * ((ei4 >> 2) & 1)) + 2 * ((ei4 >> 3) & 1);
          const uint2 qh = *(const uint2 *)fr, ql = *(const uint2 *)(fr + 256);
          const float rs = rsv[32 * (WJ * wn + j) + en];
          const unsigned uh[2] = {qh.x, qh.y}, ul[2] = {ql.x, ql.y};
#pragma unroll
          for (int c = 0; c < 4; ++c) wv[c] = dense_target_elem(v[c], fb_unsplit2_word(uh[c >> 1], ul[c >> 1], c & 1) * rs, ell);
        }
        if (pad) { wv = f32x4{0.f, 0.f, 0.f, 0.f}; ell = 0.f; }
        *(f32x4 *)(I + en * LDC + ei4) = wv;
        if constexpr (kDR) {
          cmax[j][p] = fmaxf(cmax[j][p], fmaxf(fmaxf(fabsf(wv[0]), fabsf(wv[1])), fmaxf(fabsf(wv[2]), fabsf(wv[3]))));
        } else {
#pragma unroll
          for (int c = 0; c < 4; ++c) amax[i][c] = fmaxf(amax[i][c], fabsf(wv[c]));
          const double sv = (double)wave_sum_f32(ell);
          s = p ? s + sv : sv;
        }
      }
      if constexpr (!kDR) {
        if (lane == 0) ellp[(size_t)r32[i] * ncb + cb32] = s;
      }
    }
  }
  if constexpr (kDR) {
#pragma unroll
    for (int j = 0; j < WJ; ++j)
#pragma unroll
      for (int p = 0; p < 4; ++p) {
        const float m = fb_lane_max<7>(cmax[j][p]);
        if ((lane & 7) == 0) red[w * 64 + 32 * j + 8 * p + (lane >> 3)] = m;
      }
  } else if constexpr (kSU) {
#pragma unroll
    for (int i = 0; i < 2; ++i) {
      const float m = fb_lane_max<32>(amax[i][0]);
      if (lane < 32) red[w * 64 + 32 * i + lane] = m;
    }
  } else {
#pragma unroll
    for (int i = 0; i < 2; ++i)
#pragma unroll
      for (int c = 0; c < 4; ++c) {
        const float m = fb_lane_max<56>(amax[i][c]);
        if (lane < 8) red[w * 64 + 32 * i + ei4 + c] = m;
      }
  }
  fb_barrier();
  if constexpr (kDR) {
#pragma unroll
    for (int j = 0; j < WJ; ++j) {
      const int cb32 = (col0 >> 5) + WJ * wn + j;
      float s, inv;
      fb_scale_of(fmaxf(red[wn * 64 + 32 * j + l31], red[(NWN + wn) * 64 + 32 * j + l31]), s, inv);
      if (wm == 0 && lane < 32) a.rinv[(size_t)ln * (size_t)(d >> 7) * a.M + (size_t)rb * a.M + col0 + 32 * (WJ * wn + j) + lane] = inv;
#pragma unroll
      for (int i = 0; i < 2; ++i) {
        const float *I = img + (i * WJ + j) * kImgW;
#pragma unroll
        for (int g2 = 0; g2 < 2; ++g2) {
          const f32x4 x0 = *(const f32x4 *)(I + l31 * LDC + 16 * g2 + 4 * h) * s, x1 = *(const f32x4 *)(I + l31 * LDC + 16 * g2 + 8 + 4 * h) * s;
          const float x[8] = {x0[0], x0[1], x0[2], x0[3], x1[0], x1[1], x1[2], x1[3]};
          fb_store_frag(RPl + ((size_t)cb32 * ng + 2 * r32[i] + g2) * kFrag + 4 * lane, x);
        }
      }
    }
  } else {
#pragma unroll
    for (int i = 0; i < 2; ++i) {
      float mx = red[(wm * NWN) * 64 + 32 * i + l31];
#pragma unroll
      for (int x = 1; x < NWN; ++x) mx = fmaxf(mx, red[(wm * NWN + x) * 64 + 32 * i + l31]);
      float s, inv;
      fb_scale_of(mx, s, inv);
      if (wn == 0 && lane < 32) a.winv[(size_t)ln * (size_t)(a.M >> 7) * d + (size_t)cb * d + row0 + 64 * wm + 32 * i + lane] = inv;
#pragma unroll
      for (int j = 0; j < WJ; ++j) {
        const float *I = img + (i * WJ + j) * kImgW;
        const int cb32 = (col0 >> 5) + WJ * wn + j;
#pragma unroll
        for (int g2 = 0; g2 < 2; ++g2) {
          float x[8];
#pragma unroll
          for (int e = 0; e < 8; ++e) x[e] = I[(16 * g2 + 8 * (e >> 2) + 4 * h + (e & 3)) * LDC + l31] * s;
          fb_store_frag(WVl + ((size_t)r32[i] * nmg + 2 * cb32 + g2) * kFrag + 4 * lane, x);
        }
      }
    }
  }
  FB_STAMP(a, 3);
  if (!kDG && !kSU && (flags & 1) && wn == 0 && lane < 32) {
    const int nrb = d >> 5;
#pragma unroll
    for (int i = 0; i < 2; ++i) {
      const int r = 32 * r32[i] + lane;
      float lg, bad;
      logdet_block32(r < a.dT ? a.params[a.dT + (size_t)r * a.dT + r] : 1.f, lg, bad);
      if (lane == 0) {
        a.ld_part[r32[i]] = (double)lg;
        a.ld_part[nrb + r32[i]] = (double)bad;
      }
    }
  }
}

__device__ __forceinline__ void fb_value_block(const FbArgs &a, int l, double *red) {
  const int d = a.d;
  ValueIn vin{};
  vin.ell_const = a.ell_const;
  vin.ell_part = a.ell_part + (size_t)l * a.ell_stride;
  vin.n_ell_part = (d >> 5) * (a.M >> 5);
  vin.he_part = a.he_part + (size_t)l * a.he_stride;
  vin.n_he_part = (d >> 6) * (a.M >> 5);
  vin.ld_part = a.ld_part;
  vin.n_ld_part = d >> 5;
  OutArgs out{};
  const bool last = l == a.lane_last && a.value_last;
  out.value = last ? a.value_last : a.values + (size_t)l * a.value_stride;
  if (a.parts) {
    out.partials_mode = 1;
    out.partials = a.parts + (size_t)l * a.part_stride;
    out.scalars_off = (int64_t)d + (int64_t)(d >> 7) * ((d >> 7) + 1) / 2 * 16384;
  }
  out.ent_kind = a.ent_kind;
  out.M_total = a.M_total;
  out.M_local = a.MT;
  out.status = a.status;
  const float *pp = a.params;
  const int dT = a.dT;
  finalize_value_block<float, 256, false>(dT, vin, out, (int64_t)dT + (int64_t)dT * dT, [pp, dT](int i) { return pp[dT + (size_t)i * dT + i]; }, red);
}

template <int WJ, int NRV, int TABW, int WPE, bool PART = false>
__global__ __launch_bounds__(512 / WJ, WPE / WJ) void k_fb_vjp(FbArgs a) {
  static_assert(WJ == 1, "the transposing B reads are written for the 64 x 32 wave tiles");
  constexpr int LDC = 36, NF = WJ, kPW = 2 * WJ;
  constexpr int NR = NRV;
  constexpr int kBody = (NR * kStageW > 16 * kImgW / 2) ? NR * kStageW : 16 * kImgW / 2;
  __shared__ __attribute__((aligned(16))) unsigned lds[kBody + TABW];
  float *wf = reinterpret_cast<float *>(lds + kBody);
  const int tid = threadIdx.x, lane = tid & 63, l31 = lane & 31, h = lane >> 5;
  const int w = __builtin_amdgcn_readfirstlane(tid >> 6);
  const int wm = w / (4 / WJ), wn = w % (4 / WJ);
  if ((int)blockIdx.x < a.L) {
    if (tid < 256) fb_value_block(a, (int)blockIdx.x, reinterpret_cast<double *>(lds));
    return;
  }
  const __attribute__((address_space(4))) int *wp = (const __attribute__((address_space(4))) int *)a.work + 4 * ((int)blockIdx.x - a.L);
  const int ln = wp[0], rc = wp[1];
  const int rb = rc & 0xffff, cb = rc >> 16;
  const int d = a.d, M = a.M, nmg = M >> 4, dT = a.dT;
  const int row0 = rb * 128, col0 = cb * 128;
  const bool last = ln == a.lane_last && a.grad_last;
  float *grad = last ? a.grad_last : a.grads + (size_t)ln * a.grad_stride;
  const bool upper = a.write_upper || last;
  const int G = nmg;
  const int NB = M >> 7;
  const unsigned *sp[NF];
  unsigned btr;
  {
    const int G4 = lane >> 4, c16 = lane & 15;
    const int kgpar = G4 & 1, hq = G4 >> 1, hp = c16 & 1, half = (c16 >> 1) & 1, sl = 4 * hq + (c16 >> 2);
    btr = 16u * (unsigned)(8 * (2 * hp + kgpar) + ((sl & 7) ^ (4 * hp))) + 8u * (unsigned)half;
  }
#pragma unroll
  for (int f = 0; f < NF; ++f) {
    const int fs = NF * w + f, fr = fs & 3;
    if (fs < 4) {
      sp[f] = a.WV + (size_t)ln * a.plane_stride + ((size_t)((row0 >> 5) + fr) * nmg) * kFrag + 4 * lane;
    } else {
      const int m8 = lane >> 3, s8 = m8 >> 2, hp = (m8 >> 1) & 1, kgpar = m8 & 1, sl = 8 * s8 + ((lane & 7) ^ (4 * hp));
      sp[f] = a.epsP + (size_t)ln * a.plane_stride + ((size_t)((col0 >> 4) + 2 * fr + kgpar)) * kFrag + 4 * (sl + 32 * hp);
    }
  }
  int gi = 0;
  const int bstep_odd = (d >> 4) * kFrag - 64;
  constexpr int kMaxNBv = 16;
  float twi[kMaxNBv];
  auto load_table = [&]() {
    if (tid < 128) {
      const float *wi = a.winv + (size_t)ln * (size_t)NB * d + row0 + tid;
#pragma unroll
      for (int r = 0; r < kMaxNBv; ++r) twi[r] = wi[(size_t)(r < NB ? r : NB - 1) * d];
    }
    asm volatile("" ::: "memory");
  };
  auto build_table = [&]() {
    if (tid < 128) {
      float u = twi[0], grow = 1.f;
#pragma unroll
      for (int r = 1; r < kMaxNBv; ++r) {
        if (r < NB) {
          float ratio = u / twi[r];
          if (!(ratio <= 1099511627776.f)) ratio = 1099511627776.f;
          if (ratio > 1.f && grow * ratio > 1.2089258e24f) ratio = fmaxf(1.2089258e24f / grow, 1.f);
          if (ratio > 1.f) grow *= ratio;
          wf[(r - 1) * 128 + tid] = ratio;
          u = u / ratio;
        }
      }
      wf[(NB - 1) * 128 + tid] = u;
    }
  };
  auto issue = [&](int slot) {
#pragma unroll
    for (int f = 0; f < NF; ++f) {
      unsigned *dst = lds + slot * kStageW + (NF * w + f) * 512;
      if (!(FB_VK & 16)) {
        FB_GLDS16(sp[f], dst, 0);
        FB_GLDS16(sp[f], dst, 1024);
      }
      if (NF * w + f >= 4) sp[f] += (gi & 1) ? bstep_odd : 64;
      else sp[f] += kFrag;
    }
    ++gi;
  };
  auto read_frags = [&](int slot, FbFrags<WJ> &F) {
    if ((FB_VK & 64)) return;
    const unsigned *cur = lds + slot * kStageW + 4 * lane;
#pragma unroll
    for (int i = 0; i < 2; ++i)
#pragma unroll
      for (int p = 0; p < 2; ++p) F.A[i][p] = *(const u32x4v *)(cur + ((2 * wm + i) * 2 + p) * 256);
    const unsigned bb = (unsigned)(uintptr_t)(lds + slot * kStageW) + (8 + 2 * wn) * 1024 + btr;
    uint2 t0, t1, t2, t3;
    asm volatile("ds_read_b64_tr_b16 %0, %4\n\tds_read_b64_tr_b16 %1, %4 offset:512\n\tds_read_b64_tr_b16 %2, %4 offset:1024\n\t"
                 "ds_read_b64_tr_b16 %3, %4 offset:1536\n\ts_waitcnt lgkmcnt(0)"
                 : "=&v"(t0), "=&v"(t1), "=&v"(t2), "=&v"(t3) : "v"(bb) : "memory");
    F.B[0][0] = u32x4v{t0.x, t0.y, t1.x, t1.y};
    F.B[0][1] = u32x4v{t2.x, t2.y, t3.x, t3.y};
  };
  const int ri[2] = {(row0 >> 5) + 2 * wm, (row0 >> 5) + 2 * wm + 1};
  int cj[WJ];
#pragma unroll
  for (int j = 0; j < WJ; ++j) cj[j] = (col0 >> 5) + WJ * wn + j;
  const bool work = cj[0] <= ri[1];
  bool dg[2];
#pragma unroll
  for (int i = 0; i < 2; ++i) {
    dg[i] = false;
#pragma unroll
    for (int j = 0; j < WJ; ++j) dg[i] = dg[i] || ri[i] == cj[j];
  }
  f32x16 acc[2][WJ];
#pragma unroll
  for (int i = 0; i < 2; ++i)
#pragma unroll
    for (int j = 0; j < WJ; ++j)
#pragma unroll
      for (int r = 0; r < 16; ++r) acc[i][j][r] = 0.f;
  double rsd[2] = {0.0, 0.0};
  float rcur[2] = {0.f, 0.f};
  auto after_group = [&](auto S, int g, const FbFrags<WJ> &F) {
    if (__builtin_expect(dg[0] || dg[1], 0)) {
#pragma unroll
      for (int i = 0; i < 2; ++i)
        if (dg[i]) {
#pragma unroll
          for (int e = 0; e < 8; ++e) rcur[i] += fb_unsplit2(F.A[i][0], F.A[i][1], e);
        }
    }
    if constexpr (decltype(S)::value == 3 || decltype(S)::value == -1) {
      if (((g + 1) & 7) == 0 && g + 1 < G) {
        const float *wr = wf + ((g >> 3) << 7) + 64 * wm;
#pragma unroll
        for (int i = 0; i < 2; ++i) {
#pragma unroll
          for (int q = 0; q < 4; ++q) {
            const f32x4 f4 = *(const f32x4 *)(wr + 32 * i + 8 * q + 4 * h);
#pragma unroll
            for (int j = 0; j < WJ; ++j)
#pragma unroll
              for (int c = 0; c < 4; ++c) acc[i][j][4 * q + c] *= f4[c];
          }
          rsd[i] = (rsd[i] + (double)rcur[i]) * (double)wr[32 * i + l31];
          rcur[i] = 0.f;
        }
        asm volatile("" ::: "memory");
      }
    }
  };
  auto compute = [&](auto S, int g, const FbFrags<WJ> &F) {
    if (!(FB_VK & 32)) fb_group<WJ>(F, acc);
    after_group(S, g, F);
  };
  {
    FB_STAMP(a, 0);
    FB_NOTE(a, 4, G);
    load_table();
#pragma unroll
    for (int s0 = 0; s0 < NR - 1; ++s0) issue(s0);
    fb_wait_vm<kPW * (NR - 1)>();
    build_table();
    int slot = 0;
    for (int g = 0; g < G; ++g) {
      if (g == 1) FB_STAMP(a, 1);
      if (g + NR - 2 < G) fb_wait_vm<kPW * (NR - 2)>();
      else if (NR > 3 && g + 1 < G) fb_wait_vm<kPW>();
      else fb_wait_vm<0>();
      fb_barrier();
      if (g + NR - 1 < G) issue(slot == 0 ? NR - 1 : slot - 1);
      if (work) {
        FbFrags<WJ> F;
        read_frags(slot, F);
        compute(std::integral_constant<int, -1>{}, g, F);
      }
      slot = slot == NR - 1 ? 0 : slot + 1;
    }
  }
  fb_barrier();
  FB_STAMP(a, 2);
  if ((FB_VK & 128)) return;
  float *Cs = reinterpret_cast<float *>(lds) + w * kImgW;
  const float *wfin = wf + (NB - 1) * 128 + 64 * wm;
  const double invM = 1.0 / (double)a.M_total;
  const bool pow2M = (a.M_total & (a.M_total - 1)) == 0;
  const float invMe = (float)invM * kEpsInv;
  const double direct = direct_entropy_coeff(a.ent_kind);
  const int i4 = 4 * (lane & 7);
#pragma unroll
  for (int i = 0; i < 2; ++i) {
#pragma unroll
    for (int j = 0; j < WJ; ++j) {
      if (cj[j] > ri[i] || 32 * ri[i] >= dT) continue;
      const bool diag = ri[i] == cj[j];
      const int rbase = 32 * ri[i], cbase = 32 * cj[j];
#pragma unroll
      for (int q = 0; q < 4; ++q) {
        const f32x4 v = {acc[i][j][4 * q], acc[i][j][4 * q + 1], acc[i][j][4 * q + 2], acc[i][j][4 * q + 3]};
        *(f32x4 *)(Cs + l31 * LDC + 8 * q + 4 * h) = v;
      }
      const f32x4 ff = *(const f32x4 *)(wfin + 32 * i + i4);
#pragma unroll
      for (int p = 0; p < 4; ++p) {
        const int n = 8 * p + (lane >> 3);
        const int gi = rbase + i4, gj = cbase + n;
        float cjj = 1.f;
        if (diag && gj >= gi && gj < gi + 4) cjj = a.params[dT + (size_t)gj * dT + gj];
        const f32x4 v = *(const f32x4 *)(Cs + n * LDC + i4) * ff;
        f32x4 o;
        if constexpr (PART) {
          o = v * kEpsInv;
          if (diag) {
#pragma unroll
            for (int c = 0; c < 4; ++c) o[c] = gj > gi + c ? 0.f : o[c];
          }
          store16_wt(a.parts + (size_t)ln * a.part_stride + d + ((size_t)(rb * (rb + 1) / 2 + cb) << 14) + (size_t)(gj - col0) * 128 + (gi - row0), o);
          continue;
        }
        if (!diag && pow2M) {
          o = -v * invMe;
        } else {
#pragma unroll
          for (int c = 0; c < 4; ++c) o[c] = vjp_elem(v[c] * kEpsInv, gi + c, gj, pow2M, (float)invM, invM, direct, cjj);
        }
        store16_wt(grad + dT + (size_t)gj * dT + gi, o);
      }
      if (!PART && !diag && upper) {
        const f32x4 z4 = {0.f, 0.f, 0.f, 0.f};
#pragma unroll
        for (int p = 0; p < 4; ++p) {
          const int ii = 8 * p + (lane >> 3);
          store16_wt(grad + dT + (size_t)(rbase + ii) * dT + cbase + i4, z4);
        }
      }
      asm volatile("s_waitcnt lgkmcnt(0)" ::: "memory");
    }
    if (dg[i] && 32 * ri[i] < dT) {
      const double mine = (rsd[i] + (double)rcur[i]) * (double)wfin[32 * i + l31];
      const double sm = mine + __shfl_xor(mine, 32, 64);
      if constexpr (PART) {
        if (lane < 32) a.parts[(size_t)ln * a.part_stride + 32 * ri[i] + lane] = (float)sm;
      } else {
        if (lane < 32) grad[32 * ri[i] + lane] = dmu_elem(sm, invM);
      }
    }
  }
  FB_STAMP(a, 3);
}

__global__ __launch_bounds__(256) void k_fb_finalize_parts(FbArgs a) {
  __shared__ double red[4 * 4];
  const int d = a.d, l = blockIdx.y, j = blockIdx.x, tid = threadIdx.x;
  const float *P = a.parts + (size_t)l * a.part_stride;
  const bool last = l == a.lane_last && a.grad_last;
  float *grad = last ? a.grad_last : a.grads + (size_t)l * a.grad_stride;
  const bool upper = a.write_upper || last;
  const double invM = 1.0 / (double)a.M_total;
  const bool pow2M = (a.M_total & (a.M_total - 1)) == 0;
  const double direct = direct_entropy_coeff(a.ent_kind);
  if (j == d) {
    for (int i = tid; i < d; i += 256) grad[i] = dmu_elem((double)P[i], invM);
    double s_ld = 0.0, bad = 0.0;
    for (int i = tid; i < d; i += 256) {
      const double c = (double)a.params[d + (size_t)i * d + i];
      if (!(c > 0.0)) bad = 1.0;
      s_ld += log(c);
    }
    double v[2] = {s_ld, bad};
    block_sum_n<double, 256, 2>(v, red);
    if (tid == 0) {
      const int64_t so = (int64_t)d + (int64_t)(d >> 7) * ((d >> 7) + 1) / 2 * 16384;
      const double sum_ell = (double)P[so], s_he = (double)P[so + 1], Mt = (double)a.M_total;
      const double ent = (ent_is_closed(a.ent_kind) ? 0.5 * d * (1.0 + kLog2Pi) : s_he / Mt + 0.5 * d * kLog2Pi) + v[0];
      const double value = -(sum_ell / Mt + ent);
      float *vo = (l == a.lane_last && a.value_last) ? a.value_last : a.values + (size_t)l * a.value_stride;
      *vo = (float)value;
      int st = 0;
      if (!isfinite(value)) st |= 1;
      if (v[1] > 0.0) st |= 2;
      if (st && a.status) atomicOr(a.status, st);
    }
    return;
  }
  const int cb = j >> 7, lj = j & 127;
  const float cjj = a.params[d + (size_t)j * d + j];
  for (int i4 = 4 * tid; i4 < d; i4 += 1024) {
    f32x4 o = {0.f, 0.f, 0.f, 0.f};
    if (i4 + 3 >= j) {
      const int rb = i4 >> 7;
      const f32x4 v = *(const f32x4 *)(P + d + ((size_t)(rb * (rb + 1) / 2 + cb) << 14) + (size_t)lj * 128 + (i4 & 127));
#pragma unroll
      for (int c = 0; c < 4; ++c) o[c] = vjp_elem(v[c], i4 + c, j, pow2M, (float)invM, invM, direct, cjj);
    } else if (!upper) {
      continue;
    }
    *(f32x4 *)(grad + d + (size_t)j * d + i4) = o;
  }
}

namespace {
constexpr int kBM = 128, kBN = 128;
constexpr int kWJ = FB_WJ;
constexpr int kOwnCuTilesPerCU10 = 17;

void fb_upload(DevBuf &b, const void *src, size_t bytes) {
  if (b.bytes < bytes || !b.p) {
    if (b.p) (void)hipFree(b.p);
    (void)hipMalloc(&b.p, bytes);
    b.bytes = bytes;
  }
  (void)hipMemcpy(b.p, src, bytes, hipMemcpyHostToDevice);
}
}

static int fb_pad(int x) { return (x + 127) / 128 * 128; }
bool fb_shape_ok(const mivi_ctx *c, int M) {
  static const bool off = getenv("MIVI_BATCH_GEN3") && atoi(getenv("MIVI_BATCH_GEN3")) == 0;
  return !off && c->cfg.family == MIVI_FULLRANK && c->cfg.dtype == MIVI_F32 && c->cfg.d % 32 == 0 && M % 32 == 0 && c->cfg.d >= kBM &&
         c->cfg.d <= 2048 && M >= 128 && M <= 2048;
}
bool fb_whole_tiles(const mivi_ctx *c, int M) { return c->cfg.d % kBM == 0 && M % kBN == 0; }
size_t fb_plane_words(const mivi_ctx *c, int M) { return (size_t)fb_pad(c->cfg.d) * fb_pad(M) / 512 * kFrag; }
size_t fb_cplane_words(const mivi_ctx *c) { return (size_t)(fb_pad(c->cfg.d) / 32) * (fb_pad(c->cfg.d) / 16) * kFrag; }
size_t fb_part_len(const mivi_ctx *c) {
  const size_t d = (size_t)c->cfg.d, T = d / 128;
  return (d + T * (T + 1) / 2 * 16384 + 2 + 3) / 4 * 4;
}

const FbTab *fb_prepare(mivi_ctx *c, int M, int L) {
  FbTables &ft = c->fb;
  for (FbTab &t : ft.tab)
    if (t.L == L && t.M == M && t.prod.p && t.vjp.p) return &t;
  FbTab &t = ft.tab[ft.next_tab];
  ft.next_tab = (ft.next_tab + 1) & 3;
  invalidate_graph(c);
  (void)hipStreamSynchronize(c->stream);
  t.L = t.M = 0;
  const int d = fb_pad(c->cfg.d), nrb = d / kBM, ncb = fb_pad(M) / kBN;
  std::vector<std::vector<int4>> lists(8);
  int panel = 0;
  for (int l = 0; l < L; ++l)
    for (int cb = 0; cb < ncb; ++cb, ++panel)
      for (int rb = nrb - 1; rb >= 0; --rb) lists[panel % 8].push_back(make_int4(l, rb | (cb << 16), (l == 0 && cb == 0) ? 1 : 0, 0));
  while (true) {
    int a = 0, b = 0;
    for (int x = 1; x < 8; ++x) {
      if (lists[x].size() > lists[a].size()) a = x;
      if (lists[x].size() < lists[b].size()) b = x;
    }
    if (lists[a].size() <= lists[b].size() + 1) break;
    lists[b].push_back(lists[a].back());
    lists[a].pop_back();
  }
  for (auto &li : lists) std::stable_sort(li.begin(), li.end(), [](const int4 &p, const int4 &q) { return (p.y & 0xffff) > (q.y & 0xffff); });
  std::vector<int4> prod;
  size_t mx = 0;
  for (auto &li : lists) mx = std::max(mx, li.size());
  for (size_t i = 0; i < mx; ++i)
    for (int x = 0; x < 8; ++x)
      if (i < lists[x].size()) prod.push_back(lists[x][i]);
  std::vector<int4> flat;
  for (int l = 0; l < L; ++l)
    for (int rb = 0; rb < nrb; ++rb)
      for (int cb = 0; cb <= rb; ++cb) flat.push_back(make_int4(l, rb | (cb << 16), 0, 0));
  std::vector<int4> vjp;
  {
    const size_t n = flat.size();
    size_t pos = 0;
    std::vector<std::vector<int4>> lx(8);
    for (int x = 0; x < 8; ++x) {
      const size_t e = (n * (x + 1)) / 8;
      for (; pos < e; ++pos) lx[x].push_back(flat[pos]);
    }
    size_t m2 = 0;
    for (auto &li : lx) m2 = std::max(m2, li.size());
    for (size_t i = 0; i < m2; ++i)
      for (int x = 0; x < 8; ++x)
        if (i < lx[x].size()) vjp.push_back(lx[x][i]);
  }
  std::vector<int4> prod2;
  const size_t panel_bytes = (size_t)kBM * d * 4;
  constexpr int NG = 4, NC = 8 / NG;
  if (nrb % NG == 0 && (size_t)(nrb / NG) * panel_bytes <= (1u << 20)) {
    std::vector<std::vector<int4>> lp(8);
    int pn = 0;
    for (int l = 0; l < L; ++l)
      for (int cb = 0; cb < ncb; ++cb, ++pn)
        for (int rg = 0; rg < NG; ++rg)
          for (int r = 0; r < nrb / NG; ++r) lp[rg + NG * (pn % NC)].push_back(make_int4(l, (rg * (nrb / NG) + r) | (cb << 16), 0, 0));
    size_t m3 = 0;
    for (auto &li : lp) m3 = std::max(m3, li.size());
    for (size_t i = 0; i < m3; ++i)
      for (int x = 0; x < 8; ++x)
        if (i < lp[x].size()) prod2.push_back(lp[x][i]);
  } else {
    for (int l = 0; l < L; ++l)
      for (int cb = 0; cb < ncb; ++cb)
        for (int rb = 0; rb < nrb; ++rb) prod2.push_back(make_int4(l, rb | (cb << 16), 0, 0));
  }
  std::vector<int4> prod3;
  for (auto &li : lists) std::stable_sort(li.begin(), li.end(), [](const int4 &p, const int4 &q) { return (p.y & 0xffff) < (q.y & 0xffff); });
  for (size_t i = 0; i < mx; ++i)
    for (int x = 0; x < 8; ++x)
      if (i < lists[x].size()) prod3.push_back(lists[x][i]);
  fb_upload(t.prod, prod.data(), prod.size() * sizeof(int4));
  fb_upload(t.vjp, vjp.data(), vjp.size() * sizeof(int4));
  fb_upload(t.prod2, prod2.data(), prod2.size() * sizeof(int4));
  fb_upload(t.prod3, prod3.data(), prod3.size() * sizeof(int4));
  if (!t.prod.p || !t.vjp.p || !t.prod2.p || !t.prod3.p) return nullptr;
  t.n_prod2 = (int)prod2.size();
  t.n_prod = (int)prod.size();
  t.n_vjp = (int)vjp.size();
  t.L = L;
  t.M = M;
  return &t;
}

static FbArgs fb_args(mivi_ctx *c, const void *params, int M_true) {
  FbTables &t = c->fb;
  const int d = fb_pad(c->cfg.d), M = fb_pad(M_true);
  FbArgs a{};
  a.d = d; a.M = M;
  a.dT = c->cfg.d; a.MT = M_true;
  a.params = (const float *)params;
  a.t_mean = (const float *)c->t_mean.p;
  a.t_istd = (const float *)c->t_istd.p;
  a.CA = (unsigned *)t.CA.p;
  a.cscale = (float *)t.cscale.p;
  a.pscale = (float *)t.pscale.p;
  a.tscale = (float *)t.tscale.p;
  a.winv = (float *)t.winv.p;
  a.rinv = (float *)t.rinv.p;
  a.epsP = (unsigned *)t.epsP.p;
  a.WV = (unsigned *)t.WV.p;
  a.t_prec = (const float *)c->t_prec.p; a.dP = c->dP;
  a.PA = (unsigned *)t.PA.p;
  a.RP = (unsigned *)t.RP.p;
  a.Tinv = (const float *)t.Tinv.p;
  a.TA = (unsigned *)t.TA.p;
  a.plane_stride = (long long)fb_plane_words(c, M);
  a.ell_part = (double *)t.ell.p; a.ell_stride = (long long)(d / 32) * (M / 32);
  a.he_part = (double *)t.he.p; a.he_stride = (long long)(d / 64) * (M / 32);
  a.ld_part = (double *)t.ld.p;
  a.ent_kind = c->cfg.entropy; a.M_total = c->M_total;
  a.status = (int *)c->status.p;
  a.ell_const = c->t_const;
  return a;
}

void fb_launch_eps(mivi_ctx *c, const FbStep &s, bool with_cplanes, hipStream_t stream) {
  const int d = fb_pad(c->cfg.d), M = fb_pad(s.M), L = s.L;
  FbArgs a = fb_args(c, s.params, s.M);
  a.L = L;
  a.rng = s.rng;
  a.obj = s.obj;
  const int gx = (d / 64) * (M / 32);
  a.n_riders = with_cplanes ? (4 * (d / 32) + gx - 1) / gx : 0;
  hipLaunchKernelGGL(k_fb_eps, dim3(gx, L + a.n_riders), dim3(512), 0, stream, a);
}
void fb_launch_pplanes(mivi_ctx *c, hipStream_t stream) {
  FbArgs a = fb_args(c, nullptr, c->cfg.n_mc);
  hipLaunchKernelGGL(k_fb_pplanes, dim3(c->cfg.d / 32, 4), dim3(512), 0, stream, a);
}
void fb_launch_tplanes(mivi_ctx *c, hipStream_t stream) {
  FbArgs a = fb_args(c, nullptr, c->cfg.n_mc);
  hipLaunchKernelGGL(k_fb_tplanes, dim3(c->cfg.d / 32, 4), dim3(512), 0, stream, a);
}
void fb_launch_compute(mivi_ctx *c, const FbStep &s, hipStream_t stream, int which) {
  const FbTab &tb = *s.tab;
  FbArgs a = fb_args(c, s.params, s.M);
  a.L = s.L;
  a.grads = (float *)s.grads; a.grad_stride = s.grad_stride;
  a.values = (float *)s.values; a.value_stride = s.value_stride;
  a.grad_last = (float *)s.grad_last; a.value_last = (float *)s.value_last; a.lane_last = s.lane_last;
  a.write_upper = s.write_upper;
  a.parts = (float *)s.parts; a.part_stride = s.part_stride;
  if (s.obj) { a.ent_kind = s.ent_kind; a.M_total = s.M; }
#ifdef MIVI_DEV
  static long long *dbg_buf = nullptr;
  static const bool dbg_on = getenv("MIVI_FB_DBG") != nullptr;
  if (dbg_on && !dbg_buf) (void)hipMalloc(&dbg_buf, 2 * 8192 * 8 * sizeof(long long));
  auto dump = [&](const char *name, int n) {
    if (!dbg_on) return;
    (void)hipStreamSynchronize(stream);
    std::vector<long long> h((size_t)n * 8);
    (void)hipMemcpy(h.data(), dbg_buf, h.size() * 8, hipMemcpyDeviceToHost);
    long long t0 = h[0], t3 = 0;
    for (int i = 0; i < n; ++i) { t0 = std::min(t0, h[(size_t)i * 8]); t3 = std::max(t3, h[(size_t)i * 8 + 3]); }
    double pro = 0, loop = 0, epi = 0, pg = 0; long long gs = 0;
    for (int i = 0; i < n; ++i) { const long long *r = &h[(size_t)i * 8]; pro += r[1] - r[0]; loop += r[2] - r[1]; epi += r[3] - r[2]; gs += r[4]; }
    pg = loop / (double)gs;
    fprintf(stderr, "[fbdbg] %s: %d workgroups, span %.2f us | mean prologue %.2f us, main loop %.2f us (%.3f us per group), epilogue %.2f us | last start %.2f us\n", name, n, (t3 - t0) * 0.01, pro / n * 0.01, loop / n * 0.01, pg * 0.01, epi / n * 0.01, 0.0);
    std::vector<long long> st; for (int i = 0; i < n; ++i) st.push_back(h[(size_t)i * 8] - t0);
    std::sort(st.begin(), st.end());
    fprintf(stderr, "[fbdbg]   starts (us): p25 %.2f p50 %.2f p75 %.2f p90 %.2f max %.2f\n", st[n / 4] * 0.01, st[n / 2] * 0.01, st[3 * n / 4] * 0.01, st[9 * n / 10] * 0.01, st[n - 1] * 0.01);
  };
  a.dbg = dbg_on ? dbg_buf : nullptr;
  a.knock = getenv("MIVI_FB_KNOCK") ? atoi(getenv("MIVI_FB_KNOCK")) : 0;
#endif
  a.work = (const int4 *)tb.prod.p; a.n_work = tb.n_prod;
  const int n_cu = c->n_cu > 0 ? c->n_cu : 256;
  auto own_cu_for = [&](int n, bool equal_tiles) {
#ifdef MIVI_DEV
    static const int force_ring = getenv("MIVI_FB_RING") ? atoi(getenv("MIVI_FB_RING")) : 0;
    if (force_ring == 4) return false;
    if (force_ring == 8) return true;
#endif
    const int gmax = fb_pad(c->cfg.d) / 16;
    const int thr10 = gmax <= 32 ? 10 : (gmax <= 64 ? 10 + (gmax - 32) * 7 / 32 : kOwnCuTilesPerCU10 + (gmax - 64 < 64 ? gmax - 64 : 64) * 5 / 64);
    return !equal_tiles && n > n_cu && 10 * (long long)n <= (long long)thr10 * n_cu;
  };
  auto prod = [&](auto MODE, int n) {
    constexpr int md = decltype(MODE)::value;
    if (own_cu_for(n, md == FB_DENSE_G)) hipLaunchKernelGGL((k_fb_prod<kWJ, md, 8>), dim3(n), dim3(512 / kWJ), 0, stream, a);
    else hipLaunchKernelGGL((k_fb_prod<kWJ, md, 4>), dim3(n), dim3(512 / kWJ), 0, stream, a);
  };
  if (s.dense) {
    if (which & 1) prod(std::integral_constant<int, FB_DENSE_R>{}, tb.n_prod);
    a.work = (const int4 *)tb.prod2.p; a.n_work = tb.n_prod2;
    if (which & 4) prod(std::integral_constant<int, FB_DENSE_G>{}, tb.n_prod2);
  } else if (which & 1) {
    prod(std::integral_constant<int, FB_DIAG>{}, tb.n_prod);
#ifdef MIVI_DEV
    dump("k_fb_prod<DIAG>", tb.n_prod);
#endif
  }
  if (s.stl && (which & 8)) {
    a.work = (const int4 *)tb.prod3.p; a.n_work = tb.n_prod;
    prod(std::integral_constant<int, FB_STL_U>{}, tb.n_prod);
  }
  a.work = (const int4 *)tb.vjp.p; a.n_work = tb.n_vjp;
  if (s.values_only) {
    if (which & 2) hipLaunchKernelGGL((k_fb_vjp<kWJ, 3, 256, 6>), dim3(s.L), dim3(512 / kWJ), 0, stream, a);
    return;
  }
  if (which & 2) {
    if (s.parts) {
      if (a.M <= 256) hipLaunchKernelGGL((k_fb_vjp<kWJ, 3, 256, 6, true>), dim3(tb.n_vjp + s.L), dim3(512 / kWJ), 0, stream, a);
      else hipLaunchKernelGGL((k_fb_vjp<kWJ, 3, 2048, 4, true>), dim3(tb.n_vjp + s.L), dim3(512 / kWJ), 0, stream, a);
    }
    else if (a.M <= 256) hipLaunchKernelGGL((k_fb_vjp<kWJ, 3, 256, 6>), dim3(tb.n_vjp + s.L), dim3(512 / kWJ), 0, stream, a);
    else hipLaunchKernelGGL((k_fb_vjp<kWJ, 3, 2048, 4>), dim3(tb.n_vjp + s.L), dim3(512 / kWJ), 0, stream, a);
#ifdef MIVI_DEV
    dump("k_fb_vjp", tb.n_vjp);
#endif
  }
}

void fb_launch_finalize_parts(mivi_ctx *c, const FbStep &s, hipStream_t stream) {
  FbArgs a = fb_args(c, s.params, s.M);
  a.L = s.L;
  a.grads = (float *)s.grads; a.grad_stride = s.grad_stride;
  a.values = (float *)s.values; a.value_stride = s.value_stride;
  a.grad_last = (float *)s.grad_last; a.value_last = (float *)s.value_last; a.lane_last = s.lane_last;
  a.write_upper = s.write_upper;
  a.parts = (float *)s.parts; a.part_stride = s.part_stride;
  hipLaunchKernelGGL(k_fb_finalize_parts, dim3(c->cfg.d + 1, s.L), dim3(256), 0, stream, a);
}

}
```

advancedvi.jl_amd/csrc/mivi_internal.h:

```cpp
#pragma once
#include <hip/hip_runtime.h>
#include <math.h>
#include <stdint.h>

#include <string>
#include <vector>

#include "../../include/mivi.h"
#include "philox.h"

namespace mivi {

constexpr double kLog2Pi = 1.8378770664093454835606594728112;

struct RngArgs {
  uint64_t seed;
  uint64_t idx_base;
  const uint64_t *idx_ptr;
  int m_offset;
};

enum TargetKind : int {
  TGT_NONE = 0,
  TGT_DIAG_GAUSS = 1,
  TGT_DENSE_GAUSS = 2,
  TGT_LOGREG = 3,
  TGT_FUNNEL = 4,
  TGT_CALLBACK = 5
};

struct FunnelFin {
  const double *ab;
  int n_part;
  const void *params;
  RngArgs rng;
  int d4, M;
  double sigma_v;
  const void *row0;
  const unsigned *wait_word;
  unsigned wait_val;
  int wait_n, wait_budget;
  double *mirror;
  const double *mirror_src;
  int mirror_n;
};

struct ValueIn {
  FunnelFin fn;
  const double *ell_part;
  int n_ell_part;
  const double *ell_part2;
  int n_ell_part2;
  const void *ell;
  int n_ell;
  const double *he_part;
  int n_he_part;
  const double *ld_part;
  int n_ld_part;
  double ell_const;
};

struct OutArgs {
  void *grad;
  void *value;
  void *partials;
  int partials_mode;
  long long scalars_off;
  int ent_kind;
  int M_total;
  int M_local;
  int *status;
  double *elbo_rec;
  int rec_slot;
  const void *p2p_direct;
  int p2p_gi, p2p_v;
};
struct P2PDirectTab {
  char *stage[8];
  long long n;
  int R, rank, GV, pad;
  const unsigned *ctr;
};

struct FusedUpdate {
  int rule = -1;
  void *params;
  void *state;
  const long long *t_ptr;
  long long t_base;
  double eta, b1, b2, eps, clip_eps;
  int do_clip = 0;
};

template <typename T>
struct MfArgs {
  int d;
  int M;
  int n_cc;
  int cols_per_cc;
  const T *params;
  RngArgs rng;
  int target;
  const T *t_mean;
  const T *t_istd;
  const T *G;
  int want_grad;
  double *row_part;
  double *sc_part;
  ValueIn vin;
  OutArgs out;
  long long *dbg;
  int has_prev;
  ValueIn prev_vin;
  OutArgs prev_out;
};

template <typename T>
struct SampleArgs {
  int d, M;
  const T *params;
  RngArgs rng;
  T *Z;
  T *eps;
  int ld_eps;
  T *epsT;
  int ld_epsT;
  double *he_part;
};

template <typename T>
struct FrArgs {
  int d, M, dP, MP;
  const T *params;
  const T *eps;
  const T *epsT;
  T *Z;
  T *W;
  T *RT;
  int fused_target;
  const T *t_mean;
  const T *t_istd;
  const T *t_prec;
  double *ell_part;
  double *ld_part;
  ValueIn vin;
  OutArgs out;
  long long *dbg;
  const int2 *work_tab;
  int n_work;
  int n_pre;
  SampleArgs<T> next_eps;
  ValueIn prev_vin;
  OutArgs prev_out;
  FusedUpdate upd;
  const T *adam_cc;
};

struct ValueJob {
  ValueIn vin;
  OutArgs out;
};
struct EpsJob {
  RngArgs rng;
  int parity;
};

template <typename T>
struct ColTargetArgs {
  int d, M, kind;
  const T *Z;
  T *G;
  T *ell;
  const T *t_mean;
  const T *t_istd;
  double sigma_v;
  int want_grad;
  int constrained;
};

struct DevBuf {
  void *p = nullptr;
  size_t bytes = 0;
};

struct FbTab {
  DevBuf prod, vjp, prod2, prod3;
  int n_prod = 0, n_vjp = 0, n_prod2 = 0, L = 0, M = 0;
};
struct FbTables {
  FbTab tab[4];
  int next_tab = 0;
  DevBuf CA, epsP, WV, ell, he, ld, grads, values;
  DevBuf cscale, pscale, tscale, winv, rinv;
  DevBuf PA, RP;
  bool PA_valid = false;
  DevBuf Tinv, TA, Eye;
  DevBuf parts;
  int cap_L = 0, cap_M = 0, cap_LR = 0, cap_LP = 0;
};
struct FbStep {
  const void *params;
  int M, L;
  RngArgs rng;
  void *grads; long long grad_stride;
  void *values; long long value_stride;
  void *grad_last, *value_last;
  int lane_last;
  int write_upper;
  int dense;
  int stl;
  const FbTab *tab;
  int obj;
  int ent_kind;
  int values_only;
  void *parts; long long part_stride;
};

struct GraphCache {
  hipGraphExec_t exec = nullptr;
  int count = 0;
  const void *params = nullptr;
  void *value = nullptr;
  void *grad = nullptr;
  int kind = 0;
  double p0 = 0, p1 = 0;
  void *aux0 = nullptr, *aux1 = nullptr;
  mivi_loop_t loop{};
};

}

struct mivi_ctx {
  mivi_config_t cfg;
  hipStream_t stream = nullptr;
  hipStream_t cap_stream = nullptr;
  bool own_stream = false;
  std::string err;
  int target = mivi::TGT_NONE;
  int M_total = 0;
  size_t esize = 4;

  mivi::DevBuf t_mean, t_istd, t_prec;
  double t_const = 0.0;
  double funnel_sigma_v = 1.5;
  int funnel_constrained = 0;
  mivi::DevBuf bij_mask, bij_ld;
  void *comm = nullptr;
  int comm_rank = 0, comm_world = 1;
  mivi::DevBuf dist_P, dist_S, dist_F;
  bool bij_on = false;
  hipStream_t comm_stream = nullptr;
  hipEvent_t ev_part[2] = {nullptr, nullptr}, ev_comm[2] = {nullptr, nullptr};
  mivi::DevBuf dist_P2, dist_ring[6];
  hipStream_t comm_stream2 = nullptr;
  hipStream_t fb_comm_stream = nullptr;
  hipEvent_t fb_ev_part[2] = {nullptr, nullptr}, fb_ev_comm[2] = {nullptr, nullptr};
  int p2p_pipe_state = 1;
  int dist_route = 0;
  void *p2p_buf = nullptr;
  size_t p2p_bytes = 0;
  void *p2p_peer[8] = {nullptr, nullptr, nullptr, nullptr, nullptr, nullptr, nullptr, nullptr};
  bool p2p_opened[8] = {false, false, false, false, false, false, false, false};
  mivi::DevBuf rows_eps;
  mivi::DevBuf gen_scratch;
  mivi::DevBuf p2p_tab, p2p_ctr, p2p_scratch, p2p_direct;
  bool p2p_on = false;
  bool p2p_distinct = false;
  bool p2p_verified = false;
  int p2p_rank = 0, p2p_world = 1, p2p_G = 1, p2p_vs = 0, p2p_spin = 1 << 21;
  long long p2p_n = 0, p2p_cn = 0;
  size_t p2p_lane_bytes = 0, p2p_off_fin = 0, p2p_off_arr = 0, p2p_off_farr = 0;
  const void *lr_X = nullptr;
  const uint8_t *lr_y = nullptr;
  mivi::DevBuf lr_X_own, lr_y_own, lr_scratch, lr_part, lr_Xrm, lr_xmax, lr_XA, lr_XB, lr_ZP;
  const void *lr_X_full = nullptr;
  const uint8_t *lr_y_full = nullptr;
  int64_t lr_n_full = 0;
  double lr_likeadj_full = 1.0;
  const void *lr_Xrm_act = nullptr;
  mivi::DevBuf lr_Xsub, lr_ysub, lr_Xrm_sub, lr_idx;
  int lr_route = 0;
  int64_t lr_n = 0;
  int lr_variant = 0;
  double lr_likeadj = 1.0;
  mivi_logdensity_and_gradient_fn cb_grad = nullptr;
  mivi_logdensity_fn cb_value = nullptr;
  void *cb_user = nullptr;
  mivi_logdensity_gradient_and_hessian_fn cb_hess = nullptr;
  void *cb_hess_user = nullptr;
  std::vector<char> h_Z, h_G, h_ell;

  int cap_M = 0;
  mivi::DevBuf eps[2], epsT[2], ell_part[2], he_part[2], sc_part[2], ld_part[2];
  mivi::DevBuf tabA, tabB, tabD;
  mivi::DevBuf stl_CT, stl_Dinv;
  mivi::DevBuf stl_F;
  bool want_stl_pack = false, stl_pack_done = false;
  mivi::DevBuf stl_X;
  mivi::DevBuf lds_tabV, lds_tabV64, lds_tabS;
  int lds_nV = 0, lds_nV64 = 0, lds_nS = 0, lds_M = -1;
  bool d_idx_valid = false;
  uint64_t d_idx_expect = 0;
  mivi::DevBuf lds_tabSt;
  int lds_nSt = 0, lds_st_d = -1;
  mivi::ValueJob *defer_value = nullptr;
  bool value_deferred = false;
  int he_n[2] = {0, 0};
  int nA = 0, nB = 0, nD = 0, tab_M = -1;
  int cur = 0;
  int mf_nblk = 0;
  mivi::DevBuf Z, W, RT, ell, X;
  mivi::DevBuf row_part, status, d_idx, acc, tmp_params, tmp_out;
  mivi::DevBuf obj_vals;
  mivi::DevBuf stein_A, stein_g;
  mivi::DevBuf h2_acc;
  mivi::DevBuf dog_part;
  const uint64_t *idx_src = nullptr;
  bool pre_valid = false;
  mivi::RngArgs pre_rng{};
  int pre_M = 0, pre_parity = 0;
  int pre_capturing = 0;
  unsigned long long pre_capture_id = 0;
  long long *dbg = nullptr;
  int dP = 0, MP = 0;

  mivi::GraphCache graph;
  mivi::FbTables fb;

  int idx_stride = 1;
  bool is_child = false;
  int n_cu = 0;
  size_t lds_max = 64 * 1024;
  bool exchange_lost = false;
  int last_status_bits = 0;
  mivi::DevBuf snap;
  static constexpr int kMaxKids = 15;
  mivi_ctx *kids[kMaxKids] = {};
  int n_kids = 0;
  unsigned long long target_gen = 0, kid_gen = ~0ull;
  hipEvent_t ev_fork = nullptr, ev_join[kMaxKids] = {};
  bool dist_capture_refused = false;
  bool dist_direct = false;
  bool dist_lane4 = false;
  void *value_sink = nullptr;
  void *eps_sink = nullptr;
  void *stl_sink = nullptr;
  void *lane_sink = nullptr;
  int lane_id = 0;
  mivi::DevBuf kid_out[kMaxKids];
};

namespace mivi {

struct ValueJob;
void launch_mf_main(mivi_ctx *c, const void *params, const RngArgs &rng, int M, int want_grad, const void *G,
                    const ValueIn &vin, const OutArgs &out, const ValueJob *prev = nullptr);
void launch_mf_sgd_loop(mivi_ctx *c, void *params, void *opt_state, uint64_t idx0, long long t0, int n_steps, int rule,
                        double eta, double clip_eps, double *hist, double *elbo, void *grad_out = nullptr, void *lane_scratch = nullptr,
                        void *value_last = nullptr);
bool fr_rows_loop_ok(const mivi_ctx *c);
size_t fr_rows_eps_bytes(const mivi_ctx *c, int n_steps);
size_t fr_rows_part_bytes(const mivi_ctx *c, int n_steps);
bool launch_fr_rows_loop(mivi_ctx *c, void *params, void *opt_state, uint64_t idx0, long long t0, int n_steps, int rule, double eta, double clip_eps,
                         float *eps_all, double *hist, double *elbo, void *value, const mivi_loop_t *gen = nullptr, double *part = nullptr);
bool lr_small_loop_ok(const mivi_ctx *c);
size_t lr_small_part_bytes(const mivi_ctx *c, int n_steps);
bool launch_lr_small_loop(mivi_ctx *c, void *params, const mivi_loop_t &l, double *elbo, void *value, double *part);
bool mf_gen_loop_ok(const mivi_ctx *c, int rule);
size_t mf_gen_loop_scratch_bytes(const mivi_ctx *c, int n_steps);
bool launch_mf_gen_loop(mivi_ctx *c, void *params, const mivi_loop_t &l, double *hist, double *elbo, char *scratch);
bool fr_small_loop_ok(const mivi_ctx *c);
void launch_fr_small_loop(mivi_ctx *c, void *params, void *opt_state, uint64_t idx0, long long t0, int n_steps, int rule, double eta,
                          double clip_eps, double *elbo, void *value, const mivi_loop_t *gen = nullptr);
bool launch_mf_funnel_sgd_loop(mivi_ctx *c, void *params, void *opt_state, uint64_t idx0, long long t0, int n_steps, int rule, double eta,
                               double clip_eps, double *hist, unsigned *sync, void *pub, void *gtmp, double *elbo, void *value);
void launch_mf_funnel_loop(mivi_ctx *c, const void *params, uint64_t idx0, int n_steps, double *hist, double *elbo, void *scratch,
                           void *value, void *grad, void *lane_scratch, void *e0_tab = nullptr);
int mf_loop_lanes(const mivi_ctx *c, int n_steps);
void launch_sample_mf(mivi_ctx *c, const void *params, const RngArgs &rng, int M, void *Z, void *eps, int ld_eps,
                      double *he_part);

int launch_eps(mivi_ctx *c, const RngArgs &rng, int M);
void launch_fr_sample(mivi_ctx *c, const void *params, int M, int fused_target, void *Z, const ValueJob *prev = nullptr);
void launch_fr_vjp(mivi_ctx *c, const void *params, int M, const OutArgs &out, const EpsJob *next = nullptr,
                   const ValueJob *self = nullptr, const FusedUpdate *upd = nullptr);
int fr_ld_blocks(const mivi_ctx *c);
bool f64_valu();
void prepare_tables(mivi_ctx *c, int M);
void launch_fr_dense_target(mivi_ctx *c, int M, int want_grad);
void launch_rt_from_z(mivi_ctx *c, int M);
void launch_fr_stl(mivi_ctx *c, const void *params, int M, const void *rhs = nullptr, void *out = nullptr);
void launch_stein_outer(mivi_ctx *c, int M, void *A, double *gsum, int first, double scale);
void launch_stein_finish(mivi_ctx *c, double n, const double *gsum, const double *ell_sum, const void *ell_single, void *grad, void *logpi_avg);
void launch_stein_gsum(mivi_ctx *c, int M, double *gsum, int first);
void launch_const_hess(mivi_ctx *c, void *hess);
bool target_has_hess2(const mivi_ctx *c);
size_t target_hess2_bytes(const mivi_ctx *c);
bool target_hess2_begin(mivi_ctx *c);
void target_hess2_accumulate(mivi_ctx *c, int Mc);
void target_hess2_finish(mivi_ctx *c, int n_samples, void *hess);
int fr_sample_blocks(const mivi_ctx *c, int M);
int fr_dense_blocks(const mivi_ctx *c, int M);
int eps_blocks(const mivi_ctx *c, int M);

enum LdsReduceMode : int { R_DIAG = 0, R_DENSE_R = 1, R_DENSE_G = 2, R_PLAIN = 3 };
bool lds_path_shape_ok(const mivi_ctx *c, int M);
bool lds_prepare(mivi_ctx *c, int M);
int lds_ld_blocks(const mivi_ctx *c);
int lds_eps_blocks(const mivi_ctx *c, int M);
void launch_lds_prod32(mivi_ctx *c, const void *params, int M, bool dense, int mode, void *Z, const EpsJob *next, bool want_ld,
                       bool with_dinv = false);
int lds_prod32_tiles(const mivi_ctx *c, int M);
void launch_lds_prod64(mivi_ctx *c, const void *params, int M, bool dense, int mode, void *Z, const EpsJob *next, bool want_ld);
int lds_prod64_tiles(const mivi_ctx *c, int M);
bool lds_use_prod64(const mivi_ctx *c, int M);
int lds_prod32_eps_blocks(const mivi_ctx *c, int M);
bool lds_use_prod32(const mivi_ctx *c, int M);
struct LaneSink;
LaneSink *lane_sinks_alloc(int n);
void lane_sinks_free(LaneSink *s);
void lane_sink_reset(LaneSink *s, int lane);
int lane_sink_counts(const LaneSink *s, int lane);
bool launch_lanes_prod(mivi_ctx *c, LaneSink *s, int lanes, int which);
bool launch_lanes_vjp(mivi_ctx *c, LaneSink *s, int lanes);
struct ValueSink;
ValueSink *value_sink_alloc();
void value_sink_free(ValueSink *s);
void launch_lanes_value(mivi_ctx *c, const void *params, ValueSink *s);
struct EpsSink;
EpsSink *eps_sink_alloc();
void eps_sink_free(EpsSink *s);
void eps_sink_reset(EpsSink *s);
void launch_lanes_eps(mivi_ctx *c, EpsSink *s, int lanes);
struct StlSink;
StlSink *stl_sinks_alloc(int n);
void stl_sinks_free(StlSink *s);
void stl_sink_reset(StlSink *s, int lane);
int stl_sink_count(const StlSink *s, int lane);
bool launch_lanes_stl(mivi_ctx *c, StlSink *s, int lanes, bool with_F);
bool lds_bf16x3();
void launch_lds_vjp(mivi_ctx *c, const void *params, int M, const OutArgs &out, const ValueJob *self, const FusedUpdate *upd);
bool lds_stein_ok(const mivi_ctx *c, int M);
void launch_lds_stein_outer(mivi_ctx *c, int M, void *A, double *gsum, int first, double scale, double n, void *grad, void *logpi,
                            const ValueJob *self);
void invalidate_graph(mivi_ctx *c);

bool grid_resident(const mivi_ctx *c, const void *kernel, int block, size_t dyn_lds, long long grid);
bool fb_shape_ok(const mivi_ctx *c, int M);
bool fb_whole_tiles(const mivi_ctx *c, int M);
mivi_status_t fb_objective(mivi_ctx *c, const void *params, uint64_t idx, int lanes, int entropy, void *values);
const FbTab *fb_prepare(mivi_ctx *c, int M, int L);
size_t fb_plane_words(const mivi_ctx *c, int M);
size_t fb_cplane_words(const mivi_ctx *c);
void fb_launch_eps(mivi_ctx *c, const FbStep &s, bool with_cplanes, hipStream_t stream);
void fb_launch_pplanes(mivi_ctx *c, hipStream_t stream);
void fb_launch_tplanes(mivi_ctx *c, hipStream_t stream);
size_t fb_part_len(const mivi_ctx *c);
void fb_launch_finalize_parts(mivi_ctx *c, const FbStep &s, hipStream_t stream);
void fb_launch_compute(mivi_ctx *c, const FbStep &s, hipStream_t stream, int which = 15);

bool stl2_shape_ok(const mivi_ctx *c, int M);
void launch_stl2(mivi_ctx *c, const void *params, int M, bool dinv_done = false, const void *rhs = nullptr, void *out = nullptr,
                 bool overwrite = false);

void launch_col_target(mivi_ctx *c, int M, int want_grad);
void launch_bij_forward(mivi_ctx *c, int M);
void launch_bij_backward(mivi_ctx *c, int M, int want_grad, bool add_to_ell);
bool launch_logreg_target(mivi_ctx *c, int M, int want_grad);
int logreg_kernel_bits(const mivi_ctx *c, int M);
bool logreg_uses_mfma(const mivi_ctx *c, int M);
bool logreg_reserve(mivi_ctx *c, int M);
bool logreg_prepare_f32(mivi_ctx *c);

void launch_p2p_handover4(mivi_ctx *c, unsigned *ready, unsigned ready_val, const unsigned *const *freed, const unsigned *freed_min, int n);
void launch_p2p_exchange(mivi_ctx *c, const void *params, const void *const *P, int ring, void *value, void *grad, int phases, int lane, int lanes,
                         int count, const unsigned *ready, unsigned *freed, bool direct = false);
void launch_p2p_handover(mivi_ctx *c, unsigned *ready, unsigned ready_val, const unsigned *freed, unsigned freed_min);

void launch_finalize(mivi_ctx *c, const void *params, const void *partials, void *value, void *grad);
void launch_finalize_slice(mivi_ctx *c, const void *params, const void *sum, long long g0, long long n, void *fin);
void launch_unpack_final(mivi_ctx *c, const void *fin, void *value, void *grad);
void launch_prox(mivi_ctx *c, void *params, double stepsize, const void *dog_state, int dog_kind);
void launch_poly_average(mivi_ctx *c, void *avg, const void *params, double avg_eta, const long long *t_ptr, long long t_base);
void launch_dog_update(mivi_ctx *c, void *params, const void *grad, void *state, int kind);
bool launch_dog_update_fused(mivi_ctx *c, void *params, const void *grad, void *state, int kind, double clip_eps, void *avg,
                             double avg_eta, const long long *t_ptr, long long t_base);
void launch_logreg_gather(mivi_ctx *c, int64_t b);
void launch_value_only(mivi_ctx *c, const void *params, const ValueIn &vin, const OutArgs &out);
void launch_clip(mivi_ctx *c, void *params, double epsilon);
void launch_descent(mivi_ctx *c, void *params, const void *grad, double eta, double clip_eps = NAN);
void launch_adam(mivi_ctx *c, void *params, const void *grad, void *state, const int64_t *t_ptr, int64_t t_base,
                 double eta, double b1, double b2, double eps, double clip_eps = NAN);
void launch_cocob(mivi_ctx *c, void *params, const void *grad, void *state, double alpha, double clip_eps = (double)NAN);
void launch_bump(mivi_ctx *c, uint64_t *ctr, uint64_t by);

}
```

Before: 355,200.

## Refactor dense Gaussian target via Cholesky factor of precision and precomputed T = Lᵀ C

Replaces the dense-Gaussian target's full precision-matrix product with a factored form. It uploads the inverse Cholesky factor Li and its negated transpose, and each call precomputes T = Liᵀ·C plus a shift vector b = Liᵀ(m − μ) through a piecewise triangular product, a sum and a repack into MFMA planes. The per-sample products then use the triangular factors, so the gradient pass works only on the upper block range, and the separate prod2 work table is dropped. This trades a dense d×d product per sample for triangular products plus a per-call O(d³) precompute, which adds several kernel launches and extra scratch memory.

```diff
diff --git a/advancedvi.jl_amd/csrc/api_batch.hip b/advancedvi.jl_amd/csrc/api_batch.hip
--- a/advancedvi.jl_amd/csrc/api_batch.hip
+++ b/advancedvi.jl_amd/csrc/api_batch.hip
@@ -209,16 +209,22 @@
   if (dense) {
     if (t.cap_LR < L) {
       invalidate_graph(c);
-      if ((s = ensure(c, t.RP, (size_t)L * fb_plane_words(c, M) * 4, false)) || (s = ensure(c, t.PA, fb_cplane_words(c) * 4, false)) ||
-          (s = ensure(c, t.pscale, 2 * (size_t)d * 4, false)) || (s = ensure(c, t.rinv, (size_t)L * (d / 128) * M * 4, false)))
+      const size_t cw = fb_cplane_words(c) * 4, dd = (size_t)d * d * 4;
+      if ((s = ensure(c, t.RP, (size_t)L * fb_plane_words(c, M) * 4, false)) || (s = ensure(c, t.rinv, (size_t)L * (d / 128) * M * 4, false)) ||
+          (s = ensure(c, t.LA, cw, false)) || (s = ensure(c, t.UA, cw, false)) || (s = ensure(c, t.CB, cw, false)) ||
+          (s = ensure(c, t.lscale, 2 * (size_t)d * 4, false)) || (s = ensure(c, t.uscale, 2 * (size_t)d * 4, false)) ||
+          (s = ensure(c, t.crinv, (size_t)(d / 128) * d * 4, false)) || (s = ensure(c, t.Tslab, fb_dense_piece_count(c) * 16384 * 4, false)) ||
+          (s = ensure(c, t.Tf, dd, false)) || (s = ensure(c, t.bvec, (size_t)d * 4, false)))
         return s;
+      if (!fb_dense_pieces(c)) return fail(c, MIVI_ERR_HIP, "batch engine: work table allocation failed");
       t.cap_LR = L;
-      t.PA_valid = false;
-    }
-    if (!t.PA_valid) {
-      fb_launch_pplanes(c, c->stream);
-      t.PA_valid = true;
-    }
+      t.LA_valid = false;
+    }
+    if (!t.LA_valid) {
+      fb_launch_lplanes(c, c->stream);
+      t.LA_valid = true;
+    }
+    fb_launch_dense_T(c, params, c->stream);
   }
   const bool values_only = obj_ent >= 0 || (!grads_all && !grad_last);
   const bool stl = !values_only && (c->cfg.entropy == MIVI_ENT_STL || c->cfg.entropy == MIVI_ENT_STL_ZERO_GRAD);
diff --git a/advancedvi.jl_amd/csrc/api_core.hip b/advancedvi.jl_amd/csrc/api_core.hip
--- a/advancedvi.jl_amd/csrc/api_core.hip
+++ b/advancedvi.jl_amd/csrc/api_core.hip
@@ -173,20 +173,19 @@
   if (c->is_child) c->t_mean = c->t_istd = c->t_prec = c->status = mivi::DevBuf{};
   (void)mivi_comm_destroy(c);
   if (c->graph.exec) (void)hipGraphExecDestroy(c->graph.exec);
-  DevBuf *bufs[] = {&c->t_mean, &c->t_istd, &c->t_prec, &c->lr_X_own, &c->lr_y_own, &c->lr_scratch, &c->lr_part, &c->lr_Xrm,
+  DevBuf *bufs[] = {&c->t_mean, &c->t_istd, &c->t_prec, &c->t_li, &c->t_lit, &c->lr_X_own, &c->lr_y_own, &c->lr_scratch, &c->lr_part, &c->lr_Xrm,
                     &c->eps[0], &c->eps[1], &c->epsT[0], &c->epsT[1], &c->Z, &c->W, &c->RT, &c->ell, &c->X,
                     &c->ell_part[0], &c->ell_part[1], &c->he_part[0], &c->he_part[1], &c->row_part,
                     &c->sc_part[0], &c->sc_part[1], &c->ld_part[0], &c->ld_part[1], &c->tabA, &c->tabB, &c->tabD, &c->stl_CT, &c->stl_Dinv, &c->stl_X, &c->stl_F, &c->lr_xmax, &c->lr_XA, &c->lr_XB, &c->lr_ZP, &c->lr_Xsub, &c->lr_ysub, &c->lr_Xrm_sub, &c->lr_idx, &c->dog_part, &c->stein_A, &c->stein_g, &c->h2_acc, &c->bij_mask, &c->bij_ld, &c->dist_P, &c->dist_P2, &c->dist_ring[0], &c->dist_ring[1], &c->dist_ring[2], &c->dist_ring[3], &c->dist_ring[4], &c->dist_ring[5], &c->p2p_scratch, &c->dist_S, &c->dist_F, &c->p2p_tab, &c->p2p_ctr, &c->lds_tabV, &c->lds_tabV64, &c->lds_tabS, &c->lds_tabSt, &c->status, &c->d_idx, &c->acc, &c->tmp_params, &c->tmp_out, &c->obj_vals};
   for (DevBuf *b : bufs)
     if (b->p) (void)hipFree(b->p);
   {
-    DevBuf *fbb[] = {&c->fb.CA, &c->fb.epsP, &c->fb.WV, &c->fb.ell, &c->fb.he, &c->fb.ld, &c->fb.grads, &c->fb.values, &c->fb.PA, &c->fb.RP, &c->fb.Tinv, &c->fb.TA, &c->fb.Eye, &c->snap, &c->fb.cscale, &c->fb.pscale, &c->fb.tscale, &c->fb.winv, &c->fb.rinv, &c->p2p_direct, &c->rows_eps, &c->gen_scratch};
+    DevBuf *fbb[] = {&c->fb.CA, &c->fb.epsP, &c->fb.WV, &c->fb.ell, &c->fb.he, &c->fb.ld, &c->fb.grads, &c->fb.values, &c->fb.LA, &c->fb.UA, &c->fb.lscale, &c->fb.uscale, &c->fb.CB, &c->fb.crinv, &c->fb.Tslab, &c->fb.Tf, &c->fb.bvec, &c->fb.tpiece, &c->fb.RP, &c->fb.Tinv, &c->fb.TA, &c->fb.Eye, &c->snap, &c->fb.cscale, &c->fb.tscale, &c->fb.winv, &c->fb.rinv, &c->p2p_direct, &c->rows_eps, &c->gen_scratch};
     for (DevBuf *b : fbb)
       if (b->p) (void)hipFree(b->p);
     for (auto &tb : c->fb.tab) {
       if (tb.prod.p) (void)hipFree(tb.prod.p);
       if (tb.vjp.p) (void)hipFree(tb.vjp.p);
-      if (tb.prod2.p) (void)hipFree(tb.prod2.p);
       if (tb.prod3.p) (void)hipFree(tb.prod3.p);
     }
   }
@@ -291,9 +290,20 @@
     }
   mivi_status_t s;
   if ((s = upload_vec(c, c->t_mean, m)) || (s = upload_vec(c, c->t_prec, P))) return s;
+  if (c->cfg.dtype == MIVI_F32) {
+    std::vector<float> f((size_t)d * d), ft((size_t)d * d);
+    for (int j = 0; j < d; ++j)
+      for (int i = 0; i < d; ++i) {
+        f[(size_t)j * d + i] = (float)Li[(size_t)j * d + i];
+        ft[(size_t)i * d + j] = (float)-Li[(size_t)j * d + i];
+      }
+    if ((s = ensure(c, c->t_li, f.size() * 4, false)) || (s = ensure(c, c->t_lit, ft.size() * 4, false))) return s;
+    HIPCHK(c, hipMemcpy(c->t_li.p, f.data(), f.size() * 4, hipMemcpyHostToDevice));
+    HIPCHK(c, hipMemcpy(c->t_lit.p, ft.data(), ft.size() * 4, hipMemcpyHostToDevice));
+  }
   c->t_const = -0.5 * logdet - 0.5 * d * kLog2Pi;
   c->target = TGT_DENSE_GAUSS;
-  c->fb.PA_valid = false;
+  c->fb.LA_valid = false;
   c->cap_M = 0;
   invalidate_graph(c);
   return MIVI_OK;
diff --git a/advancedvi.jl_amd/csrc/fr_elem.h b/advancedvi.jl_amd/csrc/fr_elem.h
--- a/advancedvi.jl_amd/csrc/fr_elem.h
+++ b/advancedvi.jl_amd/csrc/fr_elem.h
@@ -8,6 +8,11 @@
   const float u = (z - tm) * tis;
   ell = __builtin_fmaf(-0.5f * u, u, ell);
   return -u * tis;
+}
+
+__device__ __forceinline__ void dense_u_elem(float u, float &ell) {
+#pragma clang fp contract(off)
+  ell = __builtin_fmaf(-0.5f * u, u, ell);
 }
 
 __device__ __forceinline__ float dense_target_elem(float pr, float r, float &ell) {
diff --git a/advancedvi.jl_amd/csrc/kernels_fullrank_batch.hip b/advancedvi.jl_amd/csrc/kernels_fullrank_batch.hip
--- a/advancedvi.jl_amd/csrc/kernels_fullrank_batch.hip
+++ b/advancedvi.jl_amd/csrc/kernels_fullrank_batch.hip
@@ -27,10 +27,15 @@
   unsigned *epsP;
   unsigned *WV;
   float *winv;
-  const float *t_prec;
-  int dP;
-  unsigned *PA;
-  float *pscale;
+  const float *t_li, *t_lit;
+  unsigned *LA;
+  unsigned *UA;
+  float *lscale, *uscale;
+  unsigned *CB;
+  float *crinv;
+  float *Tslab;
+  float *Tf;
+  float *bvec;
   unsigned *RP;
   float *rinv;
   const float *Tinv;
@@ -123,9 +128,8 @@
     fb_store_frag(planes + ((size_t)rb * ng + kg) * kFrag + 4 * lane, x);
   }
 }
-__device__ __forceinline__ void fb_cplanes_block(const FbArgs &a, int rb, int sub, int nsub, float *red) {
+__device__ __forceinline__ void fb_cplanes_block(const FbArgs &a, const float *C, int rb, int sub, int nsub, float *red) {
   const int d = a.d, ng = d >> 4, dT = a.dT;
-  const float *C = a.params + dT;
   const int hi = 2 * rb + 3 < ng - 1 ? 2 * rb + 3 : ng - 1;
   if (dT == d) {
     fb_rowblock_planes(d, rb, 0, hi, sub, nsub,
@@ -144,13 +148,86 @@
                                                return v; },
                      [C, dT](int k, int row) { if (row >= dT || k > row) return 0.f; return C[(size_t)k * dT + row]; }, a.CA, a.cscale, red);
 }
-__global__ __launch_bounds__(512) void k_fb_pplanes(FbArgs a) {
+__global__ __launch_bounds__(512) void k_fb_lplanes(FbArgs a) {
   __shared__ float red[16 * 32 + 32];
-  const float *P = a.t_prec;
-  const int dP = a.dP;
-  fb_rowblock_planes(a.d, (int)blockIdx.x, 0, (a.d >> 4) - 1, (int)blockIdx.y, (int)gridDim.y,
-                     [P, dP](int k, int row) { return *(const f32x4 *)(P + (size_t)k * dP + row); },
-                     [P, dP](int k, int row) { return P[(size_t)k * dP + row]; }, a.PA, a.pscale, red);
+  const int d = a.d, rb = (int)blockIdx.x;
+  if (blockIdx.z == 0) {
+    const float *A = a.t_li;
+    fb_rowblock_planes(d, rb, 0, 8 * ((rb >> 2) + 1) - 1, (int)blockIdx.y, (int)gridDim.y,
+                       [A, d](int k, int row) { f32x4 v = *(const f32x4 *)(A + (size_t)k * d + row);
+#pragma unroll
+                                                for (int c = 0; c < 4; ++c) v[c] = k > row + c ? 0.f : v[c];
+                                                return v; },
+                       [A, d](int k, int row) { const float v = A[(size_t)k * d + row]; return k > row ? 0.f : v; }, a.LA, a.lscale, red);
+  } else {
+    const float *A = a.t_lit;
+    fb_rowblock_planes(d, rb, 2 * (rb & ~3), (d >> 4) - 1, (int)blockIdx.y, (int)gridDim.y,
+                       [A, d](int k, int row) { f32x4 v = *(const f32x4 *)(A + (size_t)k * d + row);
+#pragma unroll
+                                                for (int c = 0; c < 4; ++c) v[c] = k >= row + c ? v[c] : 0.f;
+                                                return v; },
+                       [A, d](int k, int row) { const float v = A[(size_t)k * d + row]; return k >= row ? v : 0.f; }, a.UA, a.uscale, red);
+  }
+}
+__host__ __device__ __forceinline__ int fb_piece_slot(int rb, int cb, int kb) {
+  return rb * (rb + 1) * (rb + 2) / 6 + cb * (rb + 1) - cb * (cb - 1) / 2 + (kb - cb);
+}
+__global__ __launch_bounds__(256) void k_fb_cbplanes(FbArgs a) {
+  __shared__ double part[4][64];
+  const int d = a.d, ng = d >> 4, nb = d >> 7, tid = threadIdx.x, w = tid >> 6, lane = tid & 63;
+  const int n_items = (d >> 5) * nb;
+  if ((int)blockIdx.x * 4 >= n_items) {
+    const int r64 = (int)blockIdx.x - n_items / 4, row = 64 * r64 + lane;
+    const int q = 16 * (r64 + 1);
+    const float *A = a.t_li;
+    double s = 0.0;
+    for (int k = w * q; k < (w + 1) * q; ++k) s += (double)A[(size_t)k * d + row] * ((double)a.params[k] - (double)a.t_mean[k]);
+    part[w][lane] = s;
+    __syncthreads();
+    if (w == 0) a.bvec[row] = (float)(((part[0][lane] + part[1][lane]) + part[2][lane]) + part[3][lane]);
+    return;
+  }
+  const int item = (int)blockIdx.x * 4 + w, cb32 = item / nb, b = item % nb;
+  if (b < (cb32 >> 2)) return;
+  const int l31 = lane & 31, h = lane >> 5, col = 32 * cb32 + l31;
+  const float *C = a.params + d + (size_t)col * d;
+  f32x4 v[16];
+  float m = 0.f;
+#pragma unroll
+  for (int f = 0; f < 16; ++f) {
+    const int k = 128 * b + 16 * (f >> 1) + 8 * (f & 1) + 4 * h;
+    v[f] = *(const f32x4 *)(C + k);
+#pragma unroll
+    for (int c = 0; c < 4; ++c) {
+      v[f][c] = k + c < col ? 0.f : v[f][c];
+      m = fmaxf(m, fabsf(v[f][c]));
+    }
+  }
+  m = fmaxf(m, __shfl_xor(m, 32, 64));
+  float sc, inv;
+  fb_scale_of(m, sc, inv);
+  if (h == 0) a.crinv[(size_t)b * d + col] = inv;
+#pragma unroll
+  for (int f = 0; f < 8; ++f) {
+    const f32x4 x0 = v[2 * f] * sc, x1 = v[2 * f + 1] * sc;
+    const float x[8] = {x0[0], x0[1], x0[2], x0[3], x1[0], x1[1], x1[2], x1[3]};
+    fb_store_frag(a.CB + ((size_t)cb32 * ng + 8 * b + f) * kFrag + 4 * lane, x);
+  }
+}
+__global__ __launch_bounds__(256) void k_fb_tsum(FbArgs a) {
+  const int t = (int)blockIdx.x >> 4, d = a.d;
+  int rb = 0;
+  while ((rb + 1) * (rb + 2) / 2 <= t) ++rb;
+  const int cb = t - rb * (rb + 1) / 2;
+  const int e = (((int)blockIdx.x & 15) * 256 + (int)threadIdx.x) * 4;
+  const float *src = a.Tslab + (size_t)fb_piece_slot(rb, cb, cb) * 16384 + e;
+  f32x4 s = *(const f32x4 *)src;
+  for (int kb = cb + 1; kb <= rb; ++kb) s += *(const f32x4 *)(src + (size_t)(kb - cb) * 16384);
+  *(f32x4 *)(a.Tf + (size_t)(128 * cb + (e >> 7)) * d + 128 * rb + (e & 127)) = s;
+}
+__global__ __launch_bounds__(512) void k_fb_tdplanes(FbArgs a) {
+  __shared__ float red[16 * 32 + 32];
+  fb_cplanes_block(a, a.Tf, (a.d >> 5) - 1 - (int)blockIdx.x, (int)blockIdx.y, (int)gridDim.y, red);
 }
 __global__ __launch_bounds__(512) void k_fb_tplanes(FbArgs a) {
   __shared__ float red[16 * 32 + 32];
@@ -170,7 +247,7 @@
   const int tid = threadIdx.x, eb = blockIdx.x, d = a.d;
   if ((int)blockIdx.y < a.n_riders) {
     const int r = (int)blockIdx.y * (int)gridDim.x + eb;
-    if (r < 4 * (d >> 5)) fb_cplanes_block(a, (d >> 5) - 1 - (r >> 2), r & 3, 4, E);
+    if (r < 4 * (d >> 5)) fb_cplanes_block(a, a.params + a.dT, (d >> 5) - 1 - (r >> 2), r & 3, 4, E);
     return;
   }
   const int l = (int)blockIdx.y - a.n_riders;
@@ -224,77 +301,78 @@
   return v;
 }
 
-enum { FB_DIAG = 0, FB_DENSE_R = 1, FB_DENSE_G = 2, FB_STL_U = 3 };
+enum { FB_DIAG = 0, FB_DENSE_U = 1, FB_STL_U = 3, FB_DENSE_W = 4, FB_DENSE_T = 5 };
 template <int WJ, int MODE, int NRP>
-__global__ __launch_bounds__(512 / WJ, (MODE == 2 && NRP == 4 && WJ == 1) ? 4 : 2 / WJ) void k_fb_prod(FbArgs a) {
-  constexpr bool kDG = MODE == FB_DENSE_G, kSU = MODE == FB_STL_U, kDR = MODE == FB_DENSE_R;
+__global__ __launch_bounds__(512 / WJ, (MODE == FB_DENSE_W && NRP == 4 && WJ == 1) ? 4 : 2 / WJ) void k_fb_prod(FbArgs a) {
+  constexpr bool kDG = MODE == FB_DENSE_W, kSU = MODE == FB_STL_U, kDR = MODE == FB_DENSE_U, kDT = MODE == FB_DENSE_T;
+  constexpr bool kUp = kDG || kSU;
   constexpr int LDC = 36, NF = WJ, kPW = 2 * WJ;
   constexpr int NW = 8 / WJ, NWN = 4 / WJ;
   constexpr int kBody = (NRP * kStageW > 16 * kImgW) ? NRP * kStageW : 16 * kImgW;
   constexpr bool kTabInBody = kDG && NRP * kStageW + 2048 <= kBody;
-  constexpr int kTab = kDG ? (kTabInBody ? 128 : 2048 + 128) : 0;
+  constexpr int kTab = kDG ? (kTabInBody ? 0 : 2048) : 0;
   __shared__ __attribute__((aligned(16))) unsigned lds[kBody + 4 * 128 + NW * 64 + kTab];
   float *vec = reinterpret_cast<float *>(lds + kBody);
   float *red = vec + 4 * 128;
-  float *rsv = red + NW * 64;
-  float *tab = kTabInBody ? reinterpret_cast<float *>(lds + NRP * kStageW) : rsv + 128;
+  float *tab = kTabInBody ? reinterpret_cast<float *>(lds + NRP * kStageW) : red + NW * 64;
   const int tid = threadIdx.x, lane = tid & 63, l31 = lane & 31, h = lane >> 5;
   const int w = __builtin_amdgcn_readfirstlane(tid >> 6);
   const int wm = w / NWN, wn = w % NWN;
   const __attribute__((address_space(4))) int *wp = (const __attribute__((address_space(4))) int *)a.work + 4 * blockIdx.x;
-  const int ln = wp[0], rc = wp[1], flags = wp[2];
+  const int ln = kDT ? 0 : wp[0], rc = wp[1], flags = wp[2];
   const int rb = rc & 0xffff, cb = rc >> 16;
   const int d = a.d, ng = d >> 4;
   const int row0 = rb * 128, col0 = cb * 128;
   const int R0 = row0 >> 5;
-  const int g0 = kSU ? 2 * R0 : 0;
-  const int G = kDG ? ng : (kSU ? ng - g0 : 2 * (R0 + 4));
+  const int g0 = kUp ? 2 * R0 : (kDT ? 8 * wp[0] : 0);
+  const int G = kUp ? ng - g0 : (kDT ? 8 : 2 * (R0 + 4));
   const unsigned *sp[NF];
   int gmax[NF];
 #pragma unroll
   for (int f = 0; f < NF; ++f) {
     const int fs = NF * w + f, fr = fs & 3;
     if (fs < 4) {
-      sp[f] = (kDG ? a.PA : (kSU ? a.TA : a.CA)) + ((size_t)(R0 + fr) * ng + g0) * kFrag + 4 * lane;
-      gmax[f] = (!kDG && !kSU && 2 * (R0 + fr) + 3 < G - 1) ? 2 * (R0 + fr) + 3 : G - 1;
+      sp[f] = (kDG ? a.UA : (kSU ? a.TA : (kDT ? a.LA : a.CA))) + ((size_t)(R0 + fr) * ng + g0) * kFrag + 4 * lane;
+      gmax[f] = (!kUp && !kDT && 2 * (R0 + fr) + 3 < G - 1) ? 2 * (R0 + fr) + 3 : G - 1;
     } else {
-      sp[f] = (kDG ? a.RP : a.epsP) + (size_t)ln * a.plane_stride + ((size_t)((col0 >> 5) + fr) * ng + g0) * kFrag + 4 * lane;
+      sp[f] = (kDG ? a.RP : (kDT ? a.CB : a.epsP)) + (size_t)ln * a.plane_stride + ((size_t)((col0 >> 5) + fr) * ng + g0) * kFrag + 4 * lane;
       gmax[f] = G - 1;
     }
   }
   int gd = 0;
   constexpr int kMaxNB = 16;
-  float tv[4] = {0.f, 0.f, 0.f, 0.f}, tri[kDG ? kMaxNB : 1], trs = 0.f;
+  float tv[4] = {0.f, 0.f, 0.f, 0.f}, tri[kDG ? kMaxNB : 1];
   auto load_tables = [&]() {
     if (tid < 128) {
-      if constexpr (!kDG && !kSU) {
+      if constexpr (MODE == FB_DIAG) {
         const bool in = row0 + tid < a.dT;
         tv[0] = in ? a.params[row0 + tid] : 0.f;
         tv[1] = in ? a.t_mean[row0 + tid] : 0.f;
-        if (MODE == FB_DIAG) tv[2] = in ? a.t_istd[row0 + tid] : 0.f;
-      }
-      const float *sc = kDG ? a.pscale : (kSU ? a.tscale : a.cscale);
+        tv[2] = in ? a.t_istd[row0 + tid] : 0.f;
+      }
+      if constexpr (kDR) tv[0] = a.bvec[row0 + tid];
+      if constexpr (kDT) tv[0] = a.crinv[(size_t)wp[0] * d + col0 + tid];
+      const float *sc = kDG ? a.uscale : (kSU ? a.tscale : (kDT ? a.lscale : a.cscale));
       tv[3] = sc[d + row0 + tid];
       if constexpr (kDG) {
         const float *ri = a.rinv + (size_t)ln * (size_t)(d >> 7) * a.M + col0 + tid;
         const int NB = d >> 7;
 #pragma unroll
-        for (int b = 0; b < kMaxNB; ++b) tri[b] = ri[(size_t)(b < NB ? b : NB - 1) * a.M];
-        trs = ri[(size_t)rb * a.M];
+        for (int b = 0; b < kMaxNB; ++b) tri[b] = ri[(size_t)(rb + b < NB ? rb + b : NB - 1) * a.M];
       }
     }
     asm volatile("" ::: "memory");
   };
   auto stage_tables = [&]() {
     if (tid < 128) {
-      if constexpr (!kDG && !kSU) {
+      if constexpr (!kUp) {
         vec[tid] = tv[0];
         vec[128 + tid] = tv[1];
         if (MODE == FB_DIAG) vec[256 + tid] = tv[2];
       }
-      vec[384 + tid] = tv[3] * ((kDG) ? 1.f : kEpsInv);
+      vec[384 + tid] = tv[3] * ((kDG || kDT) ? 1.f : kEpsInv);
       if constexpr (kDG) {
-        const int NB = d >> 7;
+        const int NB = (d >> 7) - rb;
         float u = tri[0], grow = 1.f;
 #pragma unroll
         for (int b = 1; b < kMaxNB; ++b) {
@@ -308,7 +386,6 @@
           }
         }
         tab[(NB - 1) * 128 + tid] = u;
-        rsv[tid] = trs;
       }
     }
   };
@@ -330,7 +407,7 @@
 #pragma unroll
       for (int r = 0; r < 16; ++r) acc[i][j][r] = 0.f;
   const int r32[2] = {R0 + 2 * wm, R0 + 2 * wm + 1};
-  const int Gw = (kDG || kSU) ? G : 2 * r32[1] + 2;
+  const int Gw = (kUp || kDT) ? G : 2 * r32[1] + 2;
   auto after_group = [&](auto S, int g) {
     if constexpr (kDG && (decltype(S)::value & 3) == 3) {
       if (((g + 1) & 7) == 0) {
@@ -438,10 +515,10 @@
     const int lr = 64 * wm + 32 * i;
     f32x4 mu = {0.f, 0.f, 0.f, 0.f}, tm = mu, tis = mu;
     const f32x4 zf = *(const f32x4 *)(vec + 384 + lr + ei4);
-    if constexpr (!kDG && !kSU) {
-      mu = *(const f32x4 *)(vec + lr + ei4);
+    if constexpr (MODE == FB_DIAG || kDR) mu = *(const f32x4 *)(vec + lr + ei4);
+    if constexpr (MODE == FB_DIAG) {
       tm = *(const f32x4 *)(vec + 128 + lr + ei4);
-      if constexpr (MODE == FB_DIAG) tis = *(const f32x4 *)(vec + 256 + lr + ei4);
+      tis = *(const f32x4 *)(vec + 256 + lr + ei4);
     }
 #pragma unroll
     for (int j = 0; j < WJ; ++j) {
@@ -467,6 +544,15 @@
             *p = x;
             amax[i][0] = fmaxf(amax[i][0], fabsf(x));
           }
+        }
+        continue;
+      }
+      if constexpr (kDT) {
+        float *dst = a.Tslab + (size_t)flags * 16384 + (size_t)(32 * (WJ * wn + j)) * 128 + lr + ei4;
+#pragma unroll
+        for (int p = 0; p < 4; ++p) {
+          const int en = 8 * p + (lane >> 3);
+          *(f32x4 *)(dst + en * 128) = *(const f32x4 *)(I + en * LDC + ei4) * zf * vec[32 * (WJ * wn + j) + en];
         }
         continue;
       }
@@ -482,15 +568,11 @@
 #pragma unroll
           for (int c = 0; c < 4; ++c) wv[c] = diag_target_elem(z[c], tm[c], tis[c], ell);
         } else if constexpr (kDR) {
-          const f32x4 z = mu + v;
-          wv = z - tm;
+          wv = mu + v;
+#pragma unroll
+          for (int c = 0; c < 4; ++c) dense_u_elem(wv[c], ell);
         } else {
-          const unsigned *fr = RPl + ((size_t)cb32 * ng + 2 * r32[i] + (ei4 >> 4)) * kFrag + 4 * (en + 32 * ((ei4 >> 2) & 1)) + 2 * ((ei4 >> 3) & 1);
-          const uint2 qh = *(const uint2 *)fr, ql = *(const uint2 *)(fr + 256);
-          const float rs = rsv[32 * (WJ * wn + j) + en];
-          const unsigned uh[2] = {qh.x, qh.y}, ul[2] = {ql.x, ql.y};
-#pragma unroll
-          for (int c = 0; c < 4; ++c) wv[c] = dense_target_elem(v[c], fb_unsplit2_word(uh[c >> 1], ul[c >> 1], c & 1) * rs, ell);
+          wv = v;
         }
         if (pad) { wv = f32x4{0.f, 0.f, 0.f, 0.f}; ell = 0.f; }
         *(f32x4 *)(I + en * LDC + ei4) = wv;
@@ -499,15 +581,18 @@
         } else {
 #pragma unroll
           for (int c = 0; c < 4; ++c) amax[i][c] = fmaxf(amax[i][c], fabsf(wv[c]));
+        }
+        if constexpr (!kDG) {
           const double sv = (double)wave_sum_f32(ell);
           s = p ? s + sv : sv;
         }
       }
-      if constexpr (!kDR) {
+      if constexpr (!kDG) {
         if (lane == 0) ellp[(size_t)r32[i] * ncb + cb32] = s;
       }
     }
   }
+  if constexpr (kDT) return;
   if constexpr (kDR) {
 #pragma unroll
     for (int j = 0; j < WJ; ++j)
@@ -574,7 +659,7 @@
     }
   }
   FB_STAMP(a, 3);
-  if (!kDG && !kSU && (flags & 1) && wn == 0 && lane < 32) {
+  if (!kUp && !kDT && (flags & 1) && wn == 0 && lane < 32) {
     const int nrb = d >> 5;
 #pragma unroll
     for (int i = 0; i < 2; ++i) {
@@ -994,26 +1079,6 @@
       for (int x = 0; x < 8; ++x)
         if (i < lx[x].size()) vjp.push_back(lx[x][i]);
   }
-  std::vector<int4> prod2;
-  const size_t panel_bytes = (size_t)kBM * d * 4;
-  constexpr int NG = 4, NC = 8 / NG;
-  if (nrb % NG == 0 && (size_t)(nrb / NG) * panel_bytes <= (1u << 20)) {
-    std::vector<std::vector<int4>> lp(8);
-    int pn = 0;
-    for (int l = 0; l < L; ++l)
-      for (int cb = 0; cb < ncb; ++cb, ++pn)
-        for (int rg = 0; rg < NG; ++rg)
-          for (int r = 0; r < nrb / NG; ++r) lp[rg + NG * (pn % NC)].push_back(make_int4(l, (rg * (nrb / NG) + r) | (cb << 16), 0, 0));
-    size_t m3 = 0;
-    for (auto &li : lp) m3 = std::max(m3, li.size());
-    for (size_t i = 0; i < m3; ++i)
-      for (int x = 0; x < 8; ++x)
-        if (i < lp[x].size()) prod2.push_back(lp[x][i]);
-  } else {
-    for (int l = 0; l < L; ++l)
-      for (int cb = 0; cb < ncb; ++cb)
-        for (int rb = 0; rb < nrb; ++rb) prod2.push_back(make_int4(l, rb | (cb << 16), 0, 0));
-  }
   std::vector<int4> prod3;
   for (auto &li : lists) std::stable_sort(li.begin(), li.end(), [](const int4 &p, const int4 &q) { return (p.y & 0xffff) < (q.y & 0xffff); });
   for (size_t i = 0; i < mx; ++i)
@@ -1021,10 +1086,8 @@
       if (i < lists[x].size()) prod3.push_back(lists[x][i]);
   fb_upload(t.prod, prod.data(), prod.size() * sizeof(int4));
   fb_upload(t.vjp, vjp.data(), vjp.size() * sizeof(int4));
-  fb_upload(t.prod2, prod2.data(), prod2.size() * sizeof(int4));
   fb_upload(t.prod3, prod3.data(), prod3.size() * sizeof(int4));
-  if (!t.prod.p || !t.vjp.p || !t.prod2.p || !t.prod3.p) return nullptr;
-  t.n_prod2 = (int)prod2.size();
+  if (!t.prod.p || !t.vjp.p || !t.prod3.p) return nullptr;
   t.n_prod = (int)prod.size();
   t.n_vjp = (int)vjp.size();
   t.L = L;
@@ -1043,14 +1106,16 @@
   a.t_istd = (const float *)c->t_istd.p;
   a.CA = (unsigned *)t.CA.p;
   a.cscale = (float *)t.cscale.p;
-  a.pscale = (float *)t.pscale.p;
   a.tscale = (float *)t.tscale.p;
   a.winv = (float *)t.winv.p;
   a.rinv = (float *)t.rinv.p;
   a.epsP = (unsigned *)t.epsP.p;
   a.WV = (unsigned *)t.WV.p;
-  a.t_prec = (const float *)c->t_prec.p; a.dP = c->dP;
-  a.PA = (unsigned *)t.PA.p;
+  a.t_li = (const float *)c->t_li.p; a.t_lit = (const float *)c->t_lit.p;
+  a.LA = (unsigned *)t.LA.p; a.UA = (unsigned *)t.UA.p;
+  a.lscale = (float *)t.lscale.p; a.uscale = (float *)t.uscale.p;
+  a.CB = (unsigned *)t.CB.p; a.crinv = (float *)t.crinv.p;
+  a.Tslab = (float *)t.Tslab.p; a.Tf = (float *)t.Tf.p; a.bvec = (float *)t.bvec.p;
   a.RP = (unsigned *)t.RP.p;
   a.Tinv = (const float *)t.Tinv.p;
   a.TA = (unsigned *)t.TA.p;
@@ -1071,12 +1136,35 @@
   a.rng = s.rng;
   a.obj = s.obj;
   const int gx = (d / 64) * (M / 32);
-  a.n_riders = with_cplanes ? (4 * (d / 32) + gx - 1) / gx : 0;
+  a.n_riders = with_cplanes && !s.dense ? (4 * (d / 32) + gx - 1) / gx : 0;
   hipLaunchKernelGGL(k_fb_eps, dim3(gx, L + a.n_riders), dim3(512), 0, stream, a);
 }
-void fb_launch_pplanes(mivi_ctx *c, hipStream_t stream) {
+void fb_launch_lplanes(mivi_ctx *c, hipStream_t stream) {
   FbArgs a = fb_args(c, nullptr, c->cfg.n_mc);
-  hipLaunchKernelGGL(k_fb_pplanes, dim3(c->cfg.d / 32, 4), dim3(512), 0, stream, a);
+  hipLaunchKernelGGL(k_fb_lplanes, dim3(c->cfg.d / 32, 4, 2), dim3(512), 0, stream, a);
+}
+size_t fb_dense_piece_count(const mivi_ctx *c) { const size_t n = (size_t)c->cfg.d / kBM; return n * (n + 1) * (n + 2) / 6; }
+bool fb_dense_pieces(mivi_ctx *c) {
+  FbTables &t = c->fb;
+  if (t.tpiece.p && t.n_tpiece == (int)fb_dense_piece_count(c)) return true;
+  const int nrb = c->cfg.d / kBM;
+  std::vector<int4> tp;
+  for (int rb = nrb - 1; rb >= 0; --rb)
+    for (int cb = 0; cb <= rb; ++cb)
+      for (int kb = cb; kb <= rb; ++kb) tp.push_back(make_int4(kb, rb | (cb << 16), fb_piece_slot(rb, cb, kb), 0));
+  (void)hipStreamSynchronize(c->stream);
+  fb_upload(t.tpiece, tp.data(), tp.size() * sizeof(int4));
+  t.n_tpiece = t.tpiece.p ? (int)tp.size() : 0;
+  return t.tpiece.p != nullptr;
+}
+void fb_launch_dense_T(mivi_ctx *c, const void *params, hipStream_t stream) {
+  FbArgs a = fb_args(c, params, c->cfg.n_mc);
+  const int d = c->cfg.d, nb = d / kBM;
+  hipLaunchKernelGGL(k_fb_cbplanes, dim3((d / 32) * nb / 4 + d / 64), dim3(256), 0, stream, a);
+  a.work = (const int4 *)c->fb.tpiece.p; a.n_work = c->fb.n_tpiece;
+  hipLaunchKernelGGL((k_fb_prod<kWJ, FB_DENSE_T, 4>), dim3(a.n_work), dim3(512 / kWJ), 0, stream, a);
+  hipLaunchKernelGGL(k_fb_tsum, dim3(nb * (nb + 1) / 2 * 16), dim3(256), 0, stream, a);
+  hipLaunchKernelGGL(k_fb_tdplanes, dim3(d / 32, 4), dim3(512), 0, stream, a);
 }
 void fb_launch_tplanes(mivi_ctx *c, hipStream_t stream) {
   FbArgs a = fb_args(c, nullptr, c->cfg.n_mc);
@@ -1116,7 +1204,7 @@
 #endif
   a.work = (const int4 *)tb.prod.p; a.n_work = tb.n_prod;
   const int n_cu = c->n_cu > 0 ? c->n_cu : 256;
-  auto own_cu_for = [&](int n, bool equal_tiles) {
+  auto own_cu_for = [&](int n) {
 #ifdef MIVI_DEV
     static const int force_ring = getenv("MIVI_FB_RING") ? atoi(getenv("MIVI_FB_RING")) : 0;
     if (force_ring == 4) return false;
@@ -1124,17 +1212,17 @@
 #endif
     const int gmax = fb_pad(c->cfg.d) / 16;
     const int thr10 = gmax <= 32 ? 10 : (gmax <= 64 ? 10 + (gmax - 32) * 7 / 32 : kOwnCuTilesPerCU10 + (gmax - 64 < 64 ? gmax - 64 : 64) * 5 / 64);
-    return !equal_tiles && n > n_cu && 10 * (long long)n <= (long long)thr10 * n_cu;
+    return n > n_cu && 10 * (long long)n <= (long long)thr10 * n_cu;
   };
   auto prod = [&](auto MODE, int n) {
     constexpr int md = decltype(MODE)::value;
-    if (own_cu_for(n, md == FB_DENSE_G)) hipLaunchKernelGGL((k_fb_prod<kWJ, md, 8>), dim3(n), dim3(512 / kWJ), 0, stream, a);
+    if (own_cu_for(n)) hipLaunchKernelGGL((k_fb_prod<kWJ, md, 8>), dim3(n), dim3(512 / kWJ), 0, stream, a);
     else hipLaunchKernelGGL((k_fb_prod<kWJ, md, 4>), dim3(n), dim3(512 / kWJ), 0, stream, a);
   };
   if (s.dense) {
-    if (which & 1) prod(std::integral_constant<int, FB_DENSE_R>{}, tb.n_prod);
-    a.work = (const int4 *)tb.prod2.p; a.n_work = tb.n_prod2;
-    if (which & 4) prod(std::integral_constant<int, FB_DENSE_G>{}, tb.n_prod2);
+    if (which & 1) prod(std::integral_constant<int, FB_DENSE_U>{}, tb.n_prod);
+    a.work = (const int4 *)tb.prod3.p;
+    if (which & 4) prod(std::integral_constant<int, FB_DENSE_W>{}, tb.n_prod);
   } else if (which & 1) {
     prod(std::integral_constant<int, FB_DIAG>{}, tb.n_prod);
 #ifdef MIVI_DEV
diff --git a/advancedvi.jl_amd/csrc/mivi_internal.h b/advancedvi.jl_amd/csrc/mivi_internal.h
--- a/advancedvi.jl_amd/csrc/mivi_internal.h
+++ b/advancedvi.jl_amd/csrc/mivi_internal.h
@@ -184,16 +184,17 @@
 };
 
 struct FbTab {
-  DevBuf prod, vjp, prod2, prod3;
-  int n_prod = 0, n_vjp = 0, n_prod2 = 0, L = 0, M = 0;
+  DevBuf prod, vjp, prod3;
+  int n_prod = 0, n_vjp = 0, L = 0, M = 0;
 };
 struct FbTables {
   FbTab tab[4];
   int next_tab = 0;
   DevBuf CA, epsP, WV, ell, he, ld, grads, values;
-  DevBuf cscale, pscale, tscale, winv, rinv;
-  DevBuf PA, RP;
-  bool PA_valid = false;
+  DevBuf cscale, tscale, winv, rinv;
+  DevBuf LA, UA, lscale, uscale, CB, crinv, Tslab, Tf, bvec, RP, tpiece;
+  int n_tpiece = 0;
+  bool LA_valid = false;
   DevBuf Tinv, TA, Eye;
   DevBuf parts;
   int cap_L = 0, cap_M = 0, cap_LR = 0, cap_LP = 0;
@@ -241,6 +242,7 @@
   size_t esize = 4;
 
   mivi::DevBuf t_mean, t_istd, t_prec;
+  mivi::DevBuf t_li, t_lit;
   double t_const = 0.0;
   double funnel_sigma_v = 1.5;
   int funnel_constrained = 0;
@@ -453,7 +455,10 @@
 size_t fb_plane_words(const mivi_ctx *c, int M);
 size_t fb_cplane_words(const mivi_ctx *c);
 void fb_launch_eps(mivi_ctx *c, const FbStep &s, bool with_cplanes, hipStream_t stream);
-void fb_launch_pplanes(mivi_ctx *c, hipStream_t stream);
+void fb_launch_lplanes(mivi_ctx *c, hipStream_t stream);
+bool fb_dense_pieces(mivi_ctx *c);
+size_t fb_dense_piece_count(const mivi_ctx *c);
+void fb_launch_dense_T(mivi_ctx *c, const void *params, hipStream_t stream);
 void fb_launch_tplanes(mivi_ctx *c, hipStream_t stream);
 size_t fb_part_len(const mivi_ctx *c);
 void fb_launch_finalize_parts(mivi_ctx *c, const FbStep &s, hipStream_t stream);
```

After: 354,900 (median of 3 runs). No clear change (-0.1%).
